# codename0og/codename-rvc-fork-3

Hardware: AMD Instinct MI355X
Metric: 48 kHz audio samples/sec end-to-end VC (higher is better)
Workload: dtype f32 (vocoder ResBlock convs and upsamplers, HuBERT, RMVPE's U-Net convs: fp32 operands as exact bf16x3 splits on the bf16 matrix cores -- six products of order <= 2^-16 per multiply-add, fp32 accumulate; everything else fp32 / fp64)

## Files before the change

codename-rvc-fork-3_amd/csrc/conv.h:

```cpp
#pragma once
#include <vector>

#include "common.h"

namespace rvc {

struct ConvParams {
    const float *x1 = nullptr; int c1 = 0; float slope1 = 1.f; int64_t x1_bstride = 0;
    const float *x2 = nullptr; int c2 = 0; float slope2 = 1.f; int64_t x2_bstride = 0;
    int64_t l_in = 0;
    int64_t l_in2 = 0;
    const float *w = nullptr;
    const uint16_t *w16 = nullptr;
    const float *bias = nullptr;
    int64_t bias_bstride = 0;
    const float *res = nullptr;
    const float *accin = nullptr;
    float *y = nullptr;
    int64_t y_bstride = 0;
    int m_total = 0;
    int c_out = 0;
    int64_t n_cols = 0;
    int64_t l_out = 0;
    int kw = 1, dil = 1, padl = 0;
    int up_stride = 0, up_pad = 0;
    int up_interleave = 0;
    float out_scale = 1.f;
    int batch = 1;
    const uint32_t *w_wino16 = nullptr;
    const void *w_f16x2 = nullptr;
    const void *w_direct1 = nullptr;
    const void *w_winobf = nullptr;
    const float *w_wino = nullptr;
    int debug = 0;
};

struct ConcurrencyScope {
    explicit ConcurrencyScope(int hint);
    ~ConcurrencyScope();
    int saved;
};

int launch_conv(const ConvParams &p, hipStream_t stream);

bool resblock_layer_supported(int c, int k);
int launch_resblock_layer(const float *x, const float *w1, const float *b1, const float *w2, const float *b2, const float *accin,
                          float *y, int batch, int c, int64_t L, int k, int dil, float slope, float out_scale, hipStream_t stream);

bool resblock_bf_enabled();
void resblock_bf_set_enabled(bool on);
bool resblock_bf_supported(int c, int k, int dil);
bool resblock_bf_preferred(int c, int k, int tap_splits = 3);
bool resblock_bf_fits(int c, int64_t L);
size_t resblock_bf_weight_bytes(int c, int k, int tap_splits = 3);
void resblock_bf_pack_host(const float *w1, const float *w2, int c, int k, std::vector<uint16_t> *out, int tap_splits = 3);
int launch_resblock_bf(const float *x, const void *u, const float *b1, const float *b2, const float *accin, float *y, int batch, int c,
                       int64_t L, int k, int dil, float slope, float out_scale, hipStream_t stream, int tap_splits = 3);

enum Cb1Format {
    CB1_BF16W = 0,
    CB1_F16X2 = 1,
};
bool convbf1_supported(int c, int k, int dil);
bool convbf1_preferred(Cb1Format fmt, int c, int k);
bool convbf1_fits(int c, int64_t L);
size_t convbf1_weight_bytes(Cb1Format fmt, int c, int k);
int convbf1_pack_host(Cb1Format fmt, const float *w, int c, int k, std::vector<uint16_t> *out);
int launch_convbf1(Cb1Format fmt, const float *x, const void *u, const float *bias, const float *res, const float *accin, float *y, int batch,
                   int c, int64_t L, int k, int dil, float slope, float out_scale, hipStream_t stream);

bool upsbf_supported(int c_in, int c_out, int rate, int ksize, int vk);
bool upsbf_fold_noise(int nc_k);
size_t upsbf_weight_bytes(int c_in, int c_out, int rate, int vk);
void upsbf_pack_host(const float *uw, const float *nw, const float *bias, int c_in, int c_out, int rate, int ksize, int vk, int nc_k,
                     int nc_stride, std::vector<uint16_t> *out);
int launch_upsbf(const float *x, const float *har, int64_t Lh, const void *u, const float *bias, float *y, int batch, int c_in, int c_out,
                 int64_t L_in, int64_t L_out, int rate, int ksize, int pad, int vk, int64_t S, int64_t P, float slope, hipStream_t stream);

bool conv2dbf_supported(int c_in, int c_out, int H, int W, int taps);
size_t conv2dbf_weight_bytes(int c_out, int c_in);
size_t conv2dbf_workspace_bytes(int batch, int c_in, int c_out, int H, int W);
void conv2dbf_pack_host(const float *w, int c_out, int c_in, std::vector<uint16_t> *out);
int launch_conv2dbf(const float *x, const void *u, const float *bias, const float *res, float *y, int batch, int c_in, int c_out, int H, int W,
                    int relu, float *ws, size_t ws_bytes, hipStream_t stream);
int launch_conv2d_finish(const float *partial, int split, int batch, int c_out, int H, int W, const float *bias, const float *res, int relu,
                         float *y, hipStream_t stream);

static inline uint16_t bf16_rne(float f) {
    uint32_t u;
    memcpy(&u, &f, 4);
    if ((u & 0x7fffffffu) > 0x7f800000u) return (uint16_t)((u >> 16) | 0x40);
    return (uint16_t)((u + 0x7fffu + ((u >> 16) & 1u)) >> 16);
}
static inline void bf16_split_host(float v, int n_terms, uint16_t *out) {
    for (int s = 0; s < n_terms; ++s) {
        out[s] = bf16_rne(v);
        const uint32_t bits = (uint32_t)out[s] << 16;
        float f;
        memcpy(&f, &bits, 4);
        v -= f;
    }
}

bool wino_enabled();
bool wino_supported(int k, int dil);
bool wino_fits(int c_in, int c_out, int64_t L);
int launch_wino_conv(const float *x, const void *u, bool u_bf16, const float *bias, const float *res, const float *accin, float *y,
                     int batch, int c_in, int c_out, int64_t L, int k, int dil, float slope, float out_scale, hipStream_t stream);
void wino_pack_host(const float *w_host, int c_out, int c_in, int k, std::vector<float> *out);
void wino_pack_host_bf16(const float *w_host, int c_out, int c_in, int k, std::vector<uint32_t> *out);

bool winobf_enabled();
bool winobf_supported(int c_in, int c_out, int k, int dil);
bool winobf_fits(int c_in, int c_out, int64_t L);
size_t winobf_weight_bytes(int c_out, int c_in, int k);
void winobf_pack_host(const float *w_host, int c_out, int c_in, int k, std::vector<uint16_t> *out);
int launch_winobf_conv(const float *x, const void *u, const float *bias, const float *res, const float *accin, float *y, int batch,
                       int c_in, int c_out, int64_t L, int k, int dil, float slope, float out_scale, hipStream_t stream);
bool winobf2_enabled();
bool winobf2_supported(int c_in, int c_out, int k, int dil);
int launch_winobf2_conv(const float *x, const void *u, const float *bias, const float *res, const float *accin, float *y, int batch,
                        int c_in, int c_out, int64_t L, int k, int dil, float slope, float out_scale, hipStream_t stream);

void conv_pack_host(const float *w_host, int c_out, int c_in, int k, std::vector<float> *out);

}
```

codename-rvc-fork-3_amd/csrc/conv.hip:

```cpp
#include <stdlib.h>

#include <atomic>

#include "conv.h"

namespace rvc {

constexpr int CONV_CH_ALIGN = 8;
constexpr int CONV_MAX_DIL = 5;

template <int KW, int MT, int NT, int WM, int WN, int CONV_CIC, bool UP, bool WB16 = false>
__global__ void __launch_bounds__(WM *WN * 64) __attribute__((amdgpu_waves_per_eu(MT == 1 ? 2 : 3, MT == 1 ? 2 : 3)))
conv_mfma_kernel(const ConvParams p) {
    constexpr int BM = 32 * MT * WM;
    constexpr int BN = 32 * NT * WN;
    constexpr int NTH = 64 * WM * WN;
    constexpr int XW = BN + (KW - 1) * CONV_MAX_DIL;
    constexpr int XTOT = CONV_CIC * XW;
    constexpr int XN = (XTOT + NTH - 1) / NTH;
    constexpr int W4TOT = KW * CONV_CIC * BM / 4;
    constexpr int WN4 = (W4TOT + NTH - 1) / NTH;

    constexpr int WTOT = KW * CONV_CIC * BM;
    __shared__ __attribute__((aligned(16))) float ws[2 * WTOT];
// ... 231 lines not shown
            }
#pragma unroll
            for (int m = 0; m < MT; ++m)
#pragma unroll
                for (int r = 0; r < 16; ++r)
#pragma unroll
                    for (int n = 0; n < NT; ++n)
                        if (ok[n]) *reinterpret_cast<float *>(reinterpret_cast<char *>(y) + boff(m, r, n)) = acc[m][n][r] * out_scale;
        }
    } else {
        const int c_out = p.c_out, up_stride = p.up_stride, up_pad = p.up_pad;
        const int64_t n_cols = p.n_cols, l_out = p.l_out;
        const float out_scale = p.out_scale;
        const int64_t cbase = col0 + wn * NT * 32 + l31;
        const float *bsrc = bias ? bias : p.w;
        if (p.up_interleave) {
            typedef float f32x2u __attribute__((ext_vector_type(2), aligned(4)));
            typedef float f32x4u __attribute__((ext_vector_type(4), aligned(4)));
            const bool quad = (up_stride & 3) == 0;
#pragma unroll
            for (int m = 0; m < MT; ++m)
#pragma unroll
                for (int r = 0; r < 16; r += 2) {
                    const int row = m0 + wm * MT * 32 + m * 32 + mfma32_row(r, lane);
                    const int co = row / up_stride, ph = row - co * up_stride;
                    float bv = bsrc[co];
                    bv = bias ? bv : 0.f;
                    float *q = y + (int64_t)co * l_out + ph - up_pad;
#pragma unroll
                    for (int n = 0; n < NT; ++n) {
                        const int64_t col = cbase + n * 32;
                        const int64_t t = col * up_stride + ph - up_pad;
                        const float v0 = (acc[m][n][r] + bv) * out_scale, v1 = (acc[m][n][r + 1] + bv) * out_scale;
                        if (col >= n_cols) continue;
                        if (quad) {
                            if ((r & 2) == 0) {
                                const float v2 = (acc[m][n][r + 2] + bv) * out_scale, v3 = (acc[m][n][r + 3] + bv) * out_scale;
                                if (t >= 0 && t + 3 < l_out) {
                                    *reinterpret_cast<f32x4u *>(q + col * up_stride) = f32x4u{v0, v1, v2, v3};
                                } else {
                                    const float vv[4] = {v0, v1, v2, v3};
#pragma unroll
                                    for (int e = 0; e < 4; ++e)
                                        if (t + e >= 0 && t + e < l_out) q[col * up_stride + e] = vv[e];
                                }
                            }
                        } else if (t >= 0 && t + 1 < l_out) {
                            *reinterpret_cast<f32x2u *>(q + col * up_stride) = f32x2u{v0, v1};
                        } else {
                            if (t >= 0 && t < l_out) q[col * up_stride] = v0;
                            if (t + 1 >= 0 && t + 1 < l_out) q[col * up_stride + 1] = v1;
                        }
                    }
                }
            return;
        }
#pragma unroll
        for (int m = 0; m < MT; ++m)
#pragma unroll
            for (int r = 0; r < 16; ++r) {
                const int row = m0 + wm * MT * 32 + m * 32 + mfma32_row(r, lane);
                const int phase = row / c_out;
                const int co = row - phase * c_out;
                float bv = bsrc[co];
                bv = bias ? bv : 0.f;
                float *q = y + (int64_t)co * l_out + phase - up_pad;
#pragma unroll
                for (int n = 0; n < NT; ++n) {
                    const int64_t col = cbase + n * 32;
                    const int64_t t = col * up_stride + phase - up_pad;
                    if (col < n_cols && t >= 0 && t < l_out) q[col * up_stride] = (acc[m][n][r] + bv) * out_scale;
                }
            }
    }
}

static std::atomic<int> g_concurrency{1};
static thread_local int t_concurrency = 0;
static int concurrency_hint() { return t_concurrency > 0 ? t_concurrency : g_concurrency.load(std::memory_order_relaxed); }
ConcurrencyScope::ConcurrencyScope(int hint) : saved(t_concurrency) { if (hint > 0) t_concurrency = hint; }
ConcurrencyScope::~ConcurrencyScope() { t_concurrency = saved; }

template <int KW, int MT, int NT, int WM, int WN, int CIC>
static int launch_cfg(const ConvParams &p, hipStream_t stream) {
    constexpr int BM = 32 * MT * WM;
    constexpr int BN = 32 * NT * WN;
    dim3 grid((unsigned)ceil_div(p.n_cols, BN), (unsigned)(p.m_total / BM), (unsigned)p.batch);
    if (p.up_stride > 0) {
        if constexpr (KW == 2) {
            hipLaunchKernelGGL((conv_mfma_kernel<KW, MT, NT, WM, WN, CIC, true>), grid, dim3(64 * WM * WN), 0, stream, p);
        } else {
            return fail("conv: scatter mode is built for 2-tap (polyphase) kernels only, got %d taps", KW);
        }
    } else if (p.w16) {
        if constexpr ((KW == 3 && CIC == 8) || ((KW == 7 || KW == 11) && CIC == 4)) {
            hipLaunchKernelGGL((conv_mfma_kernel<KW, MT, NT, WM, WN, CIC, false, true>), grid, dim3(64 * WM * WN), 0, stream, p);
        } else {
            return fail("conv: no bf16-weight kernel for %d taps at chunk depth %d", KW, CIC);
        }
    } else {
        hipLaunchKernelGGL((conv_mfma_kernel<KW, MT, NT, WM, WN, CIC, false>), grid, dim3(64 * WM * WN), 0, stream, p);
    }
    RVC_LAUNCH_CHECK();
    return 0;
}


template <int KW, int MT, int NT, int WM, int WN>
static int launch_cic(const ConvParams &p, hipStream_t stream, int cic) {
#ifdef RVC_ABLATE
    if (cic == 4) return launch_cfg<KW, MT, NT, WM, WN, 4>(p, stream);
    return launch_cfg<KW, MT, NT, WM, WN, 8>(p, stream);
#else
    (void)cic;
    return launch_cfg<KW, MT, NT, WM, WN, (KW >= 7 ? 4 : 8)>(p, stream);
#endif
}

template <int KW>
static int launch_kw(const ConvParams &p, hipStream_t stream) {
    static const int cic_env = knob("RVC_CONV_CIC", 0);
    int cic = KW >= 7 ? 4 : 8;
    if (cic_env && !p.w16) cic = cic_env;
    if ((p.c1 % cic) || (p.c2 % cic)) cic = 8;
    if (p.m_total % 128 == 0) {
        static const int narrow_env = knob("RVC_CONV_NARROW", 1);
        const int64_t tiles = ceil_div(p.n_cols, 128) * (p.m_total / 128) * p.batch;
        if (narrow_env && tiles < 1536 && concurrency_hint() <= 1) return launch_cic<KW, 2, 1, 2, 2>(p, stream, cic);
        return launch_cic<KW, 2, 2, 2, 2>(p, stream, cic);
    }
    if (p.m_total % 64 == 0) return launch_cic<KW, 2, 2, 1, 4>(p, stream, cic);
    if (p.m_total % 32 == 0) return launch_cic<KW, 1, 4, 1, 4>(p, stream, cic);
    return fail("conv: GEMM rows (%d) must be a multiple of 32", p.m_total);
}

bool wino_enabled() {
    static const int mode = knob("RVC_WINO", 1);
    return mode != 0;
}

bool winobf_enabled() {
    static const int mode = knob("RVC_WINOBF", 1);
    return mode != 0;
}

int launch_conv(const ConvParams &p_in, hipStream_t stream) {
    const bool plain = !p_in.x2 && p_in.up_stride == 0 && p_in.bias_bstride == 0 &&
        p_in.l_in == p_in.l_out && p_in.n_cols == p_in.l_out && p_in.x1_bstride == (int64_t)p_in.c1 * p_in.l_in &&
        p_in.y_bstride == (int64_t)p_in.m_total * p_in.l_out && p_in.slope1 >= 0.f && p_in.slope1 <= 1.f && p_in.padl == (p_in.kw - 1) / 2 * p_in.dil;
    if ((p_in.w_f16x2 || p_in.w_direct1) && plain && p_in.c1 == p_in.m_total && p_in.x1 != p_in.y && convbf1_supported(p_in.c1, p_in.kw, p_in.dil) &&
        convbf1_fits(p_in.c1, p_in.l_in))
        return launch_convbf1(p_in.w_f16x2 ? CB1_F16X2 : CB1_BF16W, p_in.x1, p_in.w_f16x2 ? p_in.w_f16x2 : p_in.w_direct1, p_in.bias, p_in.res, p_in.accin,
                              p_in.y, p_in.batch, p_in.c1, p_in.l_out, p_in.kw, p_in.dil, p_in.slope1, p_in.out_scale, stream);
    if (p_in.w_winobf && plain && wino_enabled() && winobf_enabled() && winobf_supported(p_in.c1, p_in.m_total, p_in.kw, p_in.dil) &&
        winobf_fits(p_in.c1, p_in.m_total, p_in.l_in))
        return launch_winobf_conv(p_in.x1, p_in.w_winobf, p_in.bias, p_in.res, p_in.accin, p_in.y, p_in.batch, p_in.c1, p_in.m_total, p_in.l_out,
                                  p_in.kw, p_in.dil, p_in.slope1, p_in.out_scale, stream);
    if ((p_in.w_wino || p_in.w_wino16) && !p_in.x2 && p_in.up_stride == 0 && p_in.c1 == p_in.m_total && p_in.bias_bstride == 0 &&
        p_in.l_in == p_in.l_out && p_in.n_cols == p_in.l_out && p_in.x1_bstride == (int64_t)p_in.c1 * p_in.l_in &&
        p_in.y_bstride == (int64_t)p_in.m_total * p_in.l_out && p_in.c1 % 32 == 0 && p_in.slope1 >= 0.f && p_in.slope1 <= 1.f && p_in.padl == (p_in.kw - 1) / 2 * p_in.dil &&
        wino_enabled() && wino_supported(p_in.kw, p_in.dil) && wino_fits(p_in.c1, p_in.m_total, p_in.l_in))
        return launch_wino_conv(p_in.x1, p_in.w_wino16 ? (const void *)p_in.w_wino16 : (const void *)p_in.w_wino, p_in.w_wino16 != nullptr, p_in.bias, p_in.res, p_in.accin, p_in.y, p_in.batch, p_in.c1, p_in.m_total, p_in.l_out,
                                p_in.kw, p_in.dil, p_in.slope1, p_in.out_scale, stream);
    static const int dbg = knob("RVC_CONV_DEBUG", 0);
    ConvParams p = p_in;
    p.debug = dbg;
    if ((p.c1 % CONV_CH_ALIGN) || (p.c2 % CONV_CH_ALIGN) || p.c1 + p.c2 <= 0)
        return fail("conv: input channels (%d + %d) must be multiples of %d", p.c1, p.c2, CONV_CH_ALIGN);
    if (p.dil < 1 || p.dil > CONV_MAX_DIL) return fail("conv: dilation %d out of range 1..%d", p.dil, CONV_MAX_DIL);
    if (p.n_cols <= 0 || p.batch <= 0) return 0;
    if (p.up_stride == 0 && (int64_t)p.m_total * p.l_out >= ((int64_t)1 << 30))
        return fail("conv: one output slab of %d x %lld floats exceeds the 4 GB the epilogue addresses", p.m_total,
                    (long long)p.l_out);
    switch (p.kw) {
        case 1: return launch_kw<1>(p, stream);
        case 2: return launch_kw<2>(p, stream);
        case 3: return launch_kw<3>(p, stream);
        case 5: return launch_kw<5>(p, stream);
        case 7: return launch_kw<7>(p, stream);
        case 11: return launch_kw<11>(p, stream);
        default: return fail("conv: unsupported kernel size %d (1, 2, 3, 5, 7, 11)", p.kw);
    }
}

void conv_pack_host(const float *w_host, int c_out, int c_in, int k, std::vector<float> *out) {
    out->resize((size_t)c_out * c_in * k);
    for (int co = 0; co < c_out; ++co)
        for (int ci = 0; ci < c_in; ++ci)
            for (int t = 0; t < k; ++t) (*out)[((size_t)t * c_in + ci) * c_out + co] = w_host[((size_t)co * c_in + ci) * k + t];
}

}

using namespace rvc;

extern "C" int rvc_set_concurrency_hint(int utterances_in_flight) {
    if (utterances_in_flight < 1) return fail("rvc_set_concurrency_hint: need at least 1, got %d", utterances_in_flight);
    g_concurrency.store(utterances_in_flight, std::memory_order_relaxed);
    return 0;
}

extern "C" int rvc_conv1d_pack_weight(const float *w_host, int c_out, int c_in, int k, float *w_packed_dev,
                                      void *stream) {
    if (!w_host || !w_packed_dev || c_out <= 0 || c_in <= 0 || k <= 0) return fail("rvc_conv1d_pack_weight: bad argument");
    std::vector<float> packed;
    conv_pack_host(w_host, c_out, c_in, k, &packed);
    return upload_packed("rvc_conv1d_pack_weight", packed.data(), packed.size() * sizeof(float), w_packed_dev, stream);
}

extern "C" int rvc_conv1d_forward(const float *x_dev, const float *w_packed_dev, const float *bias_dev,
                                  const float *res_dev, const float *acc_dev, float *y_dev, int batch, int c_in,
                                  int c_out, int64_t length, int k, int dilation, float slope_in, float out_scale,
                                  void *stream) {
    if (!x_dev || !w_packed_dev || !y_dev) return fail("rvc_conv1d_forward: null pointer");
    if (!(k & 1)) return fail("rvc_conv1d_forward: kernel size must be odd, got %d", k);
    ConvParams p;
    p.x1 = x_dev; p.c1 = c_in; p.slope1 = slope_in; p.x1_bstride = (int64_t)c_in * length;
    p.l_in = length;
    p.w = w_packed_dev; p.bias = bias_dev; p.res = res_dev; p.accin = acc_dev;
    p.y = y_dev; p.y_bstride = (int64_t)c_out * length;
    p.m_total = c_out; p.c_out = c_out; p.n_cols = length; p.l_out = length;
    p.kw = k; p.dil = dilation; p.padl = (k - 1) / 2 * dilation;
    p.out_scale = out_scale; p.batch = batch;
    return launch_conv(p, (hipStream_t)stream);
}
```

codename-rvc-fork-3_amd/csrc/convbf1.hip:

```cpp
#include <stdlib.h>

#include <algorithm>
#include <mutex>
#include <type_traits>
#include <vector>

#include "conv.h"
#include "f16x2.h"

namespace rvc {

constexpr int CB1_NTH = 512;
constexpr int CB1_CK = 64;
constexpr int CB1_N1 = 64;

struct Cb1Bf16Taps {
    static constexpr const char *NAME = "convbf1";
    using frag = bf16x8;
    static constexpr bool PAIRS = false;
    static constexpr int PLANES = 3;
    static constexpr int TAPF = 1;
    static constexpr int NACC = 1;
    static constexpr int OUT_OPS = 24, VM_MAX = 56;
    static constexpr int tap_plane(int) { return 0; }
    static constexpr int win_plane(int i) { return 2 - i; }
    static constexpr int acc_of(int) { return 0; }
};
struct Cb1F16Pairs {
    static constexpr const char *NAME = "convh2";
    using frag = f16x8;
    static constexpr bool PAIRS = true;
    static constexpr int PLANES = 2;
    static constexpr int TAPF = 2;
    static constexpr int NACC = 2;
    static constexpr int OUT_OPS = 28, VM_MAX = 60;
    static constexpr int tap_plane(int i) { return i == 2; }
    static constexpr int win_plane(int i) { return i == 0; }
    static constexpr int acc_of(int i) { return i != 1; }
};

struct Cb1Params {
    const float *x = nullptr;
    const void *u = nullptr;
    const float *bias = nullptr;
    const float *res = nullptr;
    const float *accin = nullptr;
    float *y = nullptr;
    int64_t L = 0;
    int dil = 1;
    float slope = 1.f, out_scale = 1.f;
    int tiles_per_row = 0, n_tiles = 0, per_xcd = 0;
};

template <int KW, int C, class F>
struct Cb1Geom {
    static constexpr int NCH = C / CB1_CK;
    static constexpr int RBW = C / 128;
    static constexpr int KS = CB1_CK / 16;
    static constexpr int NGC = KW * KS;
    static constexpr int NGT = NCH * NGC;
    static constexpr int H = (KW - 1) / 2;
    static constexpr int ROWB = 2 * F::PLANES * CB1_CK + 16;
    static constexpr int XROWS = CB1_N1 + (KW - 1) * 5;
    static constexpr int X_BYTES = (XROWS + 1) * ROWB;
    static constexpr int RC32 = (XROWS + 31) / 32;
    static constexpr int NIT = (CB1_CK / 8) * RC32 / 4;
    static constexpr int IO_BYTES = C * CB1_N1 * 4;
    static constexpr int LDS_BYTES = 2 * X_BYTES + IO_BYTES;
    static constexpr int ROWBLOCKS = C / 32;
    static constexpr int CONV_BYTES = NGT * ROWBLOCKS * F::TAPF * 1024;
    static constexpr int PA = F::TAPF == 1 ? 8 : 8 / RBW;
    static_assert(C == 128 || C == 256, "square layers of 128 or 256 channels");
    static_assert((CB1_CK / 8) * RC32 % 4 == 0, "the items must divide over the four stager waves");
    static_assert(4 * NIT + F::OUT_OPS <= F::VM_MAX, "memory operations in flight per stager wave");
    static_assert(LDS_BYTES <= 163840, "LDS budget");
    static_assert((ROWB / 16) % 2 == 1, "row stride must be an odd multiple of 16 bytes");
};

template <int KW, int C, class F>
__global__ void __launch_bounds__(CB1_NTH) __attribute__((amdgpu_waves_per_eu(2, 2)))
convbf1_kernel(const Cb1Params p) {
    using GM = Cb1Geom<KW, C, F>;
    using frag = typename F::frag;
    constexpr int NCH = GM::NCH, RBW = GM::RBW, KS = GM::KS, NGC = GM::NGC, NGT = GM::NGT, H = GM::H, ROWB = GM::ROWB, NIT = GM::NIT;
    constexpr int N1 = CB1_N1, CK = CB1_CK, PA = GM::PA, PLANES = F::PLANES, TAPF = F::TAPF, NACC = F::NACC;

    extern __shared__ __attribute__((aligned(16))) unsigned char cb_smem[];
    unsigned char *const xs = cb_smem;
    float *const io_lds = reinterpret_cast<float *>(cb_smem + 2 * GM::X_BYTES);

    const int tid = threadIdx.x, lane = tid & 63;
    const int wave = __builtin_amdgcn_readfirstlane(tid >> 6);
    const int half = lane >> 5, l31 = lane & 31;
    const int d = p.dil, XR = N1 + (KW - 1) * d;
    const int64_t L = p.L;
    const unsigned L4 = (unsigned)(L * 4);
    const int num_bytes = (int)((int64_t)C * L * 4);

    const int xcd = blockIdx.x & 7, slot = blockIdx.x >> 3, nslot = gridDim.x >> 3;
    const int tile_end = (xcd + 1) * p.per_xcd < p.n_tiles ? (xcd + 1) * p.per_xcd : p.n_tiles;
    const int tile0 = xcd * p.per_xcd + slot;
    if (tile0 >= tile_end) return;
    const int my_tiles = (tile_end - tile0 + nslot - 1) / nslot;
    const int n_q = my_tiles * NCH;

    if (wave >= 4) {
        __builtin_amdgcn_s_setprio(1);
        const int sw = wave - 4;
        float xr[NIT][4];
        constexpr int RC = GM::RC32;
        const int lq = lane >> 5;
        auto x_issue = [&](int q) __attribute__((always_inline)) {
            const int tl = tile0 + (q / NCH) * nslot, ch0 = (q % NCH) * CK;
            const int bb = tl / p.tiles_per_row;
            const int xt0 = (tl - bb * p.tiles_per_row) * N1 - H * d;
            const __amdgpu_buffer_rsrc_t rs = __builtin_amdgcn_make_buffer_rsrc((void *)(p.x + (int64_t)bb * C * L), 0, num_bytes, RSRC_RAW32);
            const unsigned Lu = (unsigned)L;
            int sw_o = sw;
            asm volatile("" : "+s"(sw_o));
#pragma unroll
            for (int i = 0; i < NIT; ++i) {
                const int wi = sw_o * NIT + i, qp = wi / RC, rc = wi - qp * RC;
                const int qd = 2 * qp + lq, r = rc * 32 + l31;
                const unsigned tg = (unsigned)(xt0 + r);
                const bool ok = r < XR && tg < Lu;
                const unsigned base = (unsigned)(ch0 + 4 * qd) * L4 + tg * 4u;
#pragma unroll
                for (int e = 0; e < 4; ++e)
                    xr[i][e] = __builtin_bit_cast(float, __builtin_amdgcn_raw_buffer_load_b32(rs, (int)(ok ? base + (unsigned)e * L4 : BUF_OOB), 0, 0));
            }
        };
        const float slope = p.slope;
        auto x_write = [&](int q) __attribute__((always_inline)) {
            unsigned char *const xb = xs + (q & 1) * GM::X_BYTES;
            int sw_o = sw;
            asm volatile("" : "+s"(sw_o));
#pragma unroll
            for (int i = 0; i < NIT; ++i) {
                const int wi = sw_o * NIT + i, qp = wi / RC, rc = wi - qp * RC;
                const int qd = 2 * qp + lq, r = rc * 32 + l31;
                unsigned w[2][PLANES];
#pragma unroll
                for (int e2 = 0; e2 < 2; ++e2) {
                    const float va = xr[i][2 * e2], vb = xr[i][2 * e2 + 1];
                    const float la = __builtin_fmaxf(va, mul_np(va, slope)), lb = __builtin_fmaxf(vb, mul_np(vb, slope));
                    if constexpr (F::PAIRS) split_f16x2_np(la, lb, w[e2][0], w[e2][1]);
                    else split3_np(la, lb, w[e2]);
                }
                unsigned char *o = xb + (r < XR ? r : GM::XROWS) * ROWB + qd * 8;
#pragma unroll
                for (int s = 0; s < PLANES; ++s) *reinterpret_cast<u32x2 *>(o + s * 2 * CK) = u32x2{w[0][s], w[1][s]};
                if (i & 1) __builtin_amdgcn_sched_barrier(0);
            }
        };
        constexpr int CHUNKS = N1 / 4, RPW = 64 / CHUNKS, PASSES = C / (4 * RPW);
        constexpr int HP = 4, NHF = PASSES / HP;
        const int chunk = lane % CHUNKS, rsub = lane / CHUNKS;
        const float out_scale = p.out_scale;
        const bool l4 = (L & 3) == 0;
        const bool has_res = p.res != nullptr, has_acc = p.accin != nullptr, has_bias = p.bias != nullptr;
        const __amdgpu_buffer_rsrc_t brs = __builtin_amdgcn_make_buffer_rsrc((void *)(has_bias ? p.bias : p.y), 0, C * 4, RSRC_RAW32);
        auto out_store = [&](int tl) __attribute__((always_inline)) {
            const int bb = tl / p.tiles_per_row;
            const int64_t t0 = (int64_t)(tl - bb * p.tiles_per_row) * N1;
            const bool ok = t0 + 4 * chunk < L;
            const __amdgpu_buffer_rsrc_t yrs = __builtin_amdgcn_make_buffer_rsrc((void *)(p.y + (int64_t)bb * C * L), 0, num_bytes, RSRC_RAW32);
            const __amdgpu_buffer_rsrc_t rrs = __builtin_amdgcn_make_buffer_rsrc((void *)((has_res ? p.res : p.y) + (int64_t)bb * C * L), 0, num_bytes, RSRC_RAW32);
            const __amdgpu_buffer_rsrc_t ars = __builtin_amdgcn_make_buffer_rsrc((void *)((has_acc ? p.accin : p.y) + (int64_t)bb * C * L), 0, num_bytes, RSRC_RAW32);
            const unsigned o0 = ok ? (unsigned)(sw * RPW + rsub) * L4 + (unsigned)(t0 + 4 * chunk) * 4u : BUF_OOB;
            auto load4 = [&](const __amdgpu_buffer_rsrc_t &rsrc, unsigned o) __attribute__((always_inline)) -> f32x4 {
                if (l4) return __builtin_bit_cast(f32x4, __builtin_amdgcn_raw_buffer_load_b128(rsrc, (int)o, 0, 0));
                float ae[4];
#pragma unroll
                for (int e = 0; e < 4; ++e) {
                    const unsigned oe = (ok && t0 + 4 * chunk + e < L) ? o + 4u * (unsigned)e : BUF_OOB;
                    ae[e] = __builtin_bit_cast(float, __builtin_amdgcn_raw_buffer_load_b32(rsrc, (int)oe, 0, 0));
                }
                return f32x4{ae[0], ae[1], ae[2], ae[3]};
            };
#pragma unroll
            for (int hf = 0; hf < NHF; ++hf) {
                f32x4 v[HP], rv[HP], av[HP];
                float bv[HP];
#pragma unroll
                for (int k = 0; k < HP; ++k) {
                    const unsigned o = o0 + (unsigned)((hf * HP + k) * 4 * RPW) * L4;
                    rv[k] = f32x4{0.f, 0.f, 0.f, 0.f};
                    av[k] = f32x4{0.f, 0.f, 0.f, 0.f};
                    if constexpr (F::PAIRS)
                        bv[k] = __builtin_bit_cast(float, __builtin_amdgcn_raw_buffer_load_b32(brs, (int)(has_bias ? (unsigned)((((hf * HP + k) * 4 + sw) * RPW + rsub) * 4) : BUF_OOB), 0, 0));
                    if (has_res) rv[k] = load4(rrs, o);
                    if (has_acc) av[k] = load4(ars, o);
                }
#pragma unroll
                for (int k = 0; k < HP; ++k) v[k] = *reinterpret_cast<const f32x4 *>(io_lds + (((hf * HP + k) * 4 + sw) * RPW + rsub) * N1 + 4 * chunk);
#pragma unroll
                for (int k = 0; k < HP; ++k) {
                    const unsigned o = o0 + (unsigned)((hf * HP + k) * 4 * RPW) * L4;
                    float re[4] = {v[k].x, v[k].y, v[k].z, v[k].w};
                    const float r4[4] = {rv[k].x, rv[k].y, rv[k].z, rv[k].w}, a4[4] = {av[k].x, av[k].y, av[k].z, av[k].w};
#pragma unroll
                    for (int e = 0; e < 4; ++e) {
                        if constexpr (F::PAIRS) re[e] = add_np(re[e], bv[k]);
                        if (has_res) re[e] = add_np(re[e], r4[e]);
                        if (has_acc) re[e] = add_np(re[e], a4[e]);
                        re[e] = mul_np(re[e], out_scale);
                    }
                    if (l4) {
                        __builtin_amdgcn_raw_buffer_store_b128(__builtin_bit_cast(u32x4, f32x4{re[0], re[1], re[2], re[3]}), yrs, (int)o, 0, 0);
                    } else {
#pragma unroll
                        for (int e = 0; e < 4; ++e) {
                            const unsigned oe = (ok && t0 + 4 * chunk + e < L) ? o + 4u * (unsigned)e : BUF_OOB;
                            __builtin_amdgcn_raw_buffer_store_b32(__builtin_bit_cast(unsigned, re[e]), yrs, (int)oe, 0, 0);
                        }
                    }
                }
            }
        };
        x_issue(0);
        x_write(0);
        if (1 < n_q) x_issue(1);
        for (int q = 0; q < n_q; ++q) {
            lds_barrier();
            if (q % NCH == 0 && q > 0) out_store(tile0 + (q / NCH - 1) * nslot);
            if (q + 1 < n_q) x_write(q + 1);
            asm volatile("s_waitcnt vmcnt(8)" ::: "memory");
            if (q + 2 < n_q) x_issue(q + 2);
        }
        lds_barrier();
        out_store(tile0 + (my_tiles - 1) * nslot);
        return;
    }

    float bias[RBW][16];
    if constexpr (!F::PAIRS) {
#pragma unroll
        for (int rb = 0; rb < RBW; ++rb)
#pragma unroll
            for (int r = 0; r < 16; ++r) {
                const int ch = 32 * (RBW * wave + rb) + (r & 3) + 8 * (r >> 2) + 4 * half;
                bias[rb][r] = p.bias ? p.bias[ch] : 0.f;
            }
    }
    const __amdgpu_buffer_rsrc_t urs = __builtin_amdgcn_make_buffer_rsrc((void *)p.u, 0, GM::CONV_BYTES, RSRC_RAW32);
    frag fa[PA][RBW][TAPF];
    frag fb[2][2][PLANES];
    f32x16 acc[RBW][2][NACC];
    auto load_a = [&](int slot_a, int g) __attribute__((always_inline)) {
        const int soff = (g * GM::ROWBLOCKS + RBW * wave) * TAPF * 1024;
#pragma unroll
        for (int f = 0; f < TAPF * RBW; ++f)
            fa[slot_a][f / TAPF][f % TAPF] = __builtin_bit_cast(frag, __builtin_amdgcn_raw_buffer_load_b128(urs, 16 * lane + f * 1024, soff, 0));
    };
    auto load_a1 = [&](int slot_a, int g, int f) __attribute__((always_inline)) {
        const int soff = (g * GM::ROWBLOCKS + RBW * wave) * TAPF * 1024;
        fa[slot_a][f / TAPF][f % TAPF] = __builtin_bit_cast(frag, __builtin_amdgcn_raw_buffer_load_b128(urs, 16 * lane + f * 1024, soff, 0));
    };
    auto load_b1 = [&](int buf, const unsigned char *src, int gc, int cb, int s) __attribute__((always_inline)) {
        const int tap = gc / KS, ks = gc - tap * KS;
        fb[buf][cb][s] = __builtin_bit_cast(frag, *reinterpret_cast<const u32x4 *>(src + tap * d * ROWB + ks * 32 + cb * 32 * ROWB + s * 2 * CK));
    };
#pragma unroll
    for (int g = 0; g < PA - 1; ++g) load_a(g, g);
    const int x_lane = l31 * ROWB + half * 16;
    float *const io_mine = io_lds + (32 * RBW * wave + 4 * half) * N1 + l31;
    constexpr int NM = 6 * RBW;

    static_assert((2 * NGC) % PA == 0 && NCH % 2 == 0, "two chunks of groups must be whole turns of the tap ring");
    int q = 0;
    for (int t = 0; t < my_tiles; ++t) {
#pragma unroll
        for (int rb = 0; rb < RBW; ++rb)
#pragma unroll
            for (int cb = 0; cb < 2; ++cb)
#pragma unroll
                for (int a = 0; a < NACC; ++a)
#pragma unroll
                    for (int r = 0; r < 16; ++r) acc[rb][cb][a][r] = 0.f;
#pragma unroll 1
        for (int cp = 0; cp < NCH / 2; ++cp) {
            const int g0 = cp * 2 * NGC;
#pragma unroll
            for (int c2 = 0; c2 < 2; ++c2, ++q) {
                lds_barrier();
                const unsigned char *const src = xs + (q & 1) * GM::X_BYTES + x_lane;
#pragma unroll
                for (int k = 0; k < 2 * PLANES; ++k) load_b1(0, src, 0, k & 1, PLANES - 1 - (k >> 1));
#pragma unroll
                for (int gc = 0; gc < NGC; ++gc) {
                    const int gl = c2 * NGC + gc;
#pragma unroll
                    for (int i = 0; i < 3; ++i)
#pragma unroll
                        for (int cb = 0; cb < 2; ++cb)
#pragma unroll
                            for (int rb = 0; rb < RBW; ++rb) {
                                const int k = (2 * i + cb) * RBW + rb;
                                const int wp = F::tap_plane(i), xp = F::win_plane(i), ap = F::acc_of(i);
                                if constexpr (F::PAIRS)
                                    acc[rb][cb][ap] = __builtin_amdgcn_mfma_f32_32x32x16_f16(fa[gl % PA][rb][wp], fb[gc & 1][cb][xp], acc[rb][cb][ap], 0, 0, 0);
                                else
                                    acc[rb][cb][ap] = __builtin_amdgcn_mfma_f32_32x32x16_bf16(fa[gl % PA][rb][wp], fb[gc & 1][cb][xp], acc[rb][cb][ap], 0, 0, 0);
                                __builtin_amdgcn_sched_barrier(0);
                                if (k < 2 * PLANES && gc + 1 < NGC) load_b1((gc + 1) & 1, src, gc + 1, k & 1, PLANES - 1 - (k >> 1));
                                if (k >= NM - TAPF * RBW) {
                                    int gn = g0 + gl + PA - 1;
                                    gn = gn >= NGT ? gn - NGT : gn;
                                    load_a1((gl + PA - 1) % PA, gn, k - (NM - TAPF * RBW));
                                }
                                __builtin_amdgcn_sched_barrier(0);
                            }
                }
            }
        }
#pragma unroll
        for (int rb = 0; rb < RBW; ++rb)
#pragma unroll
            for (int cb = 0; cb < 2; ++cb)
#pragma unroll
                for (int r = 0; r < 16; ++r)
                    if constexpr (F::PAIRS)
                        io_mine[(32 * rb + (r & 3) + 8 * (r >> 2)) * N1 + cb * 32] = __builtin_fmaf(acc[rb][cb][1][r], F16X2_LO_UNSCALE, acc[rb][cb][0][r]);
                    else
                        io_mine[(32 * rb + (r & 3) + 8 * (r >> 2)) * N1 + cb * 32] = acc[rb][cb][0][r] + bias[rb][r];
    }
    lds_barrier();
}


bool convbf1_supported(int c, int k, int dil) { return (c == 128 || c == 256) && (k == 3 || k == 7 || k == 11) && dil >= 1 && dil <= 5; }

bool convbf1_preferred(Cb1Format fmt, int c, int k) {
    if (fmt == CB1_F16X2) {
#ifdef RVC_ABLATE
        static const int on = knob("RVC_CH2", 1);
        if (!on) return false;
#endif
        return convbf1_supported(c, k, 1);
    }
#ifdef RVC_ABLATE
    static const int on = knob("RVC_CB1", 1);
    if (!on) return false;
    static const int all = knob("RVC_CB1_ALL", 0);
    if (all) return true;
#endif
    return (c == 128 && k == 11) || c == 256;
}

bool convbf1_fits(int c, int64_t L) { return fits_2gib((int64_t)c * L, 4); }

size_t convbf1_weight_bytes(Cb1Format fmt, int c, int k) { return (size_t)(c / 16) * k * (c / 32) * 1024 * (fmt == CB1_F16X2 ? 2 : 1); }

int convbf1_pack_host(Cb1Format fmt, const float *w, int c, int k, std::vector<uint16_t> *out) {
    const int NCH = c / CB1_CK, KS = CB1_CK / 16, RB = c / 32, planes = fmt == CB1_F16X2 ? 2 : 1;
    if (fmt == CB1_F16X2)
        for (size_t i = 0, n = (size_t)c * c * k; i < n; ++i)
            if (!(w[i] >= -F16_MAX && w[i] <= F16_MAX)) return 1;
    out->assign(convbf1_weight_bytes(fmt, c, k) / 2, 0);
    for (int ch = 0; ch < NCH; ++ch)
        for (int tap = 0; tap < k; ++tap)
            for (int ks = 0; ks < KS; ++ks)
                for (int rb = 0; rb < RB; ++rb)
                    for (int lane = 0; lane < 64; ++lane)
                        for (int e = 0; e < 8; ++e) {
                            const int co = 32 * rb + (lane & 31), ci = CB1_CK * ch + 16 * ks + 8 * (lane >> 5) + e;
                            const size_t group = ((size_t)ch * k + tap) * KS + ks, at = (group * RB + rb) * planes * 512 + lane * 8 + e;
                            const float v = w[((size_t)co * c + ci) * k + tap];
                            if (fmt == CB1_F16X2) f16x2_split_host(v, &(*out)[at], &(*out)[at + 512]);
                            else (*out)[at] = bf16_rne(v);
                        }
    return 0;
}

template <int KW, int C, class F>
static int cb1_launch(Cb1Params p, int batch, hipStream_t stream) {
    if (reserve_whole_cu((const void *)convbf1_kernel<KW, C, F>, F::NAME)) return 1;
    p.tiles_per_row = (int)ceil_div(p.L, CB1_N1);
    p.n_tiles = p.tiles_per_row * batch;
    const PersistentGrid g = persistent_grid(p.n_tiles);
    p.per_xcd = g.per_xcd;
    hipLaunchKernelGGL((convbf1_kernel<KW, C, F>), dim3(g.blocks), dim3(CB1_NTH), LDS_WHOLE_CU, stream, p);
    RVC_LAUNCH_CHECK();
    return 0;
}

template <class F>
static int cb1_dispatch(const Cb1Params &p, int batch, int c, int k, hipStream_t stream) {
#define RVC_CB1_CASE(KW, CC) if (k == KW && c == CC) return cb1_launch<KW, CC, F>(p, batch, stream)
    RVC_CB1_CASE(3, 128); RVC_CB1_CASE(7, 128); RVC_CB1_CASE(11, 128);
    RVC_CB1_CASE(3, 256); RVC_CB1_CASE(7, 256); RVC_CB1_CASE(11, 256);
#undef RVC_CB1_CASE
    return fail("%s: unsupported shape c=%d k=%d", F::NAME, c, k);
}

int launch_convbf1(Cb1Format fmt, const float *x, const void *u, const float *bias, const float *res, const float *accin, float *y, int batch,
                   int c, int64_t L, int k, int dil, float slope, float out_scale, hipStream_t stream) {
    const char *const name = fmt == CB1_F16X2 ? Cb1F16Pairs::NAME : Cb1Bf16Taps::NAME;
    if (!convbf1_supported(c, k, dil)) return fail("%s: unsupported shape (%d channels, %d taps, dilation %d)", name, c, k, dil);
    if (x == y) return fail("%s: in-place operation is not supported", name);
    if (!(slope >= 0.f && slope <= 1.f)) return fail("%s: leaky slope %g outside [0, 1]", name, (double)slope);
    if (!convbf1_fits(c, L)) return fail("%s: a %d x %lld slab exceeds the 2 GiB buffer addressing", name, c, (long long)L);
    if (L <= 0 || batch <= 0) return 0;
    if ((int64_t)ceil_div(L, CB1_N1) * batch >= ((int64_t)1 << 28)) return fail("%s: too many tiles", name);
    Cb1Params p;
    p.x = x; p.u = u; p.bias = bias; p.res = res; p.accin = accin; p.y = y; p.L = L; p.dil = dil; p.slope = slope; p.out_scale = out_scale;
    return fmt == CB1_F16X2 ? cb1_dispatch<Cb1F16Pairs>(p, batch, c, k, stream) : cb1_dispatch<Cb1Bf16Taps>(p, batch, c, k, stream);
}

}

using namespace rvc;


static int cb1_abi_weight_bytes(Cb1Format fmt, const char *fn, int c, int k, size_t *bytes) {
    if (!bytes) return fail("%s: null pointer", fn);
    if (!convbf1_supported(c, k, 1)) return fail("%s: c must be 128 or 256, k 3, 7 or 11", fn);
    *bytes = convbf1_weight_bytes(fmt, c, k);
    return 0;
}

static int cb1_abi_pack_weight(Cb1Format fmt, const char *fn, const char *shape_fn, const float *w_host, int c, int k, void *u_dev, void *stream) {
    if (!w_host || !u_dev) return fail("%s: null pointer", fn);
    size_t bytes = 0;
    if (cb1_abi_weight_bytes(fmt, shape_fn, c, k, &bytes)) return 1;
    std::vector<uint16_t> u;
    if (convbf1_pack_host(fmt, w_host, c, k, &u)) return fail("%s: a tap is non-finite or beyond +-65504, the range of an fp16 pair", fn);
    return upload_packed(fn, u.data(), bytes, u_dev, stream);
}

static int cb1_abi_forward(Cb1Format fmt, const char *fn, const float *x_dev, const void *u_dev, const float *bias_dev, const float *res_dev,
                           const float *acc_dev, float *y_dev, int batch, int c, int64_t length, int k, int dilation, float slope_in,
                           float out_scale, void *stream) {
    if (!x_dev || !u_dev || !y_dev) return fail("%s: null pointer", fn);
    return launch_convbf1(fmt, x_dev, u_dev, bias_dev, res_dev, acc_dev, y_dev, batch, c, length, k, dilation, slope_in, out_scale,
                          (hipStream_t)stream);
}

extern "C" int rvc_conv1d_bf16w_weight_bytes(int c, int k, size_t *bytes) {
    return cb1_abi_weight_bytes(CB1_BF16W, "rvc_conv1d_bf16w_weight_bytes", c, k, bytes);
}
extern "C" int rvc_conv1d_bf16w_pack_weight(const float *w_host, int c, int k, void *u_dev, void *stream) {
    return cb1_abi_pack_weight(CB1_BF16W, "rvc_conv1d_bf16w_pack_weight", "rvc_conv1d_bf16w_weight_bytes", w_host, c, k, u_dev, stream);
}
extern "C" int rvc_conv1d_bf16w_forward(const float *x_dev, const void *u_dev, const float *bias_dev, const float *res_dev,
                                        const float *acc_dev, float *y_dev, int batch, int c, int64_t length, int k, int dilation,
                                        float slope_in, float out_scale, void *stream) {
    return cb1_abi_forward(CB1_BF16W, "rvc_conv1d_bf16w_forward", x_dev, u_dev, bias_dev, res_dev, acc_dev, y_dev, batch, c, length, k,
                           dilation, slope_in, out_scale, stream);
}

extern "C" int rvc_conv1d_f16x2_weight_bytes(int c, int k, size_t *bytes) {
    return cb1_abi_weight_bytes(CB1_F16X2, "rvc_conv1d_f16x2_weight_bytes", c, k, bytes);
}
extern "C" int rvc_conv1d_f16x2_pack_weight(const float *w_host, int c, int k, void *u_dev, void *stream) {
    return cb1_abi_pack_weight(CB1_F16X2, "rvc_conv1d_f16x2_pack_weight", "rvc_conv1d_f16x2_pack_weight", w_host, c, k, u_dev, stream);
}
extern "C" int rvc_conv1d_f16x2_forward(const float *x_dev, const void *u_dev, const float *bias_dev, const float *res_dev,
                                        const float *acc_dev, float *y_dev, int batch, int c, int64_t length, int k, int dilation,
                                        float slope_in, float out_scale, void *stream) {
    return cb1_abi_forward(CB1_F16X2, "rvc_conv1d_f16x2_forward", x_dev, u_dev, bias_dev, res_dev, acc_dev, y_dev, batch, c, length, k,
                           dilation, slope_in, out_scale, stream);
}
```

codename-rvc-fork-3_amd/csrc/decoder.h:

```cpp
#pragma once
#include <atomic>
#include <map>
#include <mutex>
#include <string>
#include <vector>

#include "conv.h"

namespace rvc {

constexpr int MRF_MAX_DIM = 9;

struct HostTensor {
    std::vector<float> data;
    std::vector<int64_t> shape;
    int64_t numel() const { int64_t n = 1; for (auto s : shape) n *= s; return n; }
};

template <typename T>
struct DevBufT {
    T *p = nullptr;
    ~DevBufT() { if (p) (void)hipFree(p); }
    int upload(const std::vector<T> &h) {
        if (p) { (void)hipFree(p); p = nullptr; }
        hipError_t e = hipMalloc((void **)&p, h.size() * sizeof(T));
        if (e == hipSuccess) e = hipMemcpy(p, h.data(), h.size() * sizeof(T), hipMemcpyHostToDevice);
        return e == hipSuccess ? 0 : fail("device upload of %zu %zu-byte values failed: %s", h.size(), sizeof(T), hipGetErrorString(e));
    }
};
using DevBuf = DevBufT<float>;
using DevBuf16 = DevBufT<uint16_t>;

struct ConvW {
    DevBuf w, b;
    DevBuf16 w16;
    DevBuf wu;
    DevBuf16 wu16;
    DevBuf16 wx;
    DevBuf16 wd;
    DevBuf16 wh;
    int c_in = 0, c_out = 0, k = 0;
};

struct Stage {
    int c_in = 0, c_out = 0, rate = 0, ksize = 0, pad = 0, opad = 0;
    int taps = 0;
    bool interleave = false;
    int nc_stride = 0, nc_k = 0, nc_pad = 0;
    int vk = 0, vk_rows = 0;
    int64_t S = 0, P = 0;
    DevBuf w, b;
    DevBuf16 wub;
    int ub_vk = 0;
    int nc_rows = 0;
    DevBuf nc_w;
    std::vector<ConvW> c1, c2;
    std::vector<DevBuf16> pair;
    int pair_splits = 3;
};

constexpr int MAX_BRANCH_LANES = 7;
struct BranchLanes {
    hipStream_t side[MAX_BRANCH_LANES] = {};
    hipEvent_t fork = nullptr;
    hipEvent_t last[MAX_BRANCH_LANES + 1] = {};
    int n_side = 0;
    int create(int n);
    ~BranchLanes();
};

struct RefineStage {
    int ch_in = 0, ch_out = 0, rate = 0, down_c = 0, down_k = 0, down_stride = 0, down_pad = 0;
    DevBuf down_w, down_b;
    ConvW input_conv;
    DevBuf adain1[4], adain2[4];
    std::vector<ConvW> c1, c2;
    std::vector<DevBuf16> pair;
};

}

struct rvc_decoder {
    rvc_decoder_config cfg;
    std::map<std::string, rvc::HostTensor> host;
    bool finalized = false;
    int arithmetic = 0;
    int upp = 1;
    int dim = 1;
    float lin_w[rvc::MRF_MAX_DIM] = {0};
    float lin_b = 0.f;
    rvc::ConvW pre;
    rvc::DevBuf cond_w, cond_b;
    std::vector<rvc::Stage> stages;
    rvc::DevBuf post_w;
    float post_b = 0.f;
    int post_cin = 0;
    float merge_w = 1.f;
    rvc::DevBuf pre_w, pre_b;
    rvc::ConvW mel;
    std::vector<rvc::RefineStage> rstages;
    std::atomic<int> concurrency{0};
    std::atomic<int> branch_parallel{0};
    std::mutex lanes_mu;
    std::map<hipStream_t, rvc::BranchLanes *> lanes;
    ~rvc_decoder() { for (auto &kv : lanes) delete kv.second; }
    int tap_stage = -2;
    float *tap_dev = nullptr;
};


namespace rvc {
const HostTensor *find(const rvc_decoder *d, const std::string &name);
int need(const rvc_decoder *d, const std::string &name, const HostTensor **out, std::vector<int64_t> shape);
int build_conv(const rvc_decoder *d, const std::string &prefix, int c_out, int c_in, int k, bool bias, ConvW *out, bool as_bf16 = false);

int launch_unfold_src(const float *har, int batch, int64_t L, int64_t S, int64_t P, int k_valid, int k_rows, int64_t nq, float *V,
                      hipStream_t stream);
int launch_cond_bias(const float *pre_b, const float *cond_w, const float *cond_b, const float *g, int batch, int gin, int c0,
                     float *out, hipStream_t stream);
int launch_conv_post(const float *x, const float *w, float bias, int batch, int c_in, int64_t L, float slope, float *out,
                     hipStream_t stream, int64_t o_lo = 0, int64_t n_out = -1);

int refine_finalize(rvc_decoder *d);
size_t refine_workspace_bytes(const rvc_decoder *d, int batch, int64_t T);
int refine_forward(rvc_decoder *d, const float *z_dev, const float *f0_dev, const float *g_dev, const rvc_decoder_noise *noise,
                   int batch, int64_t T, float *out_dev, void *workspace_dev, size_t workspace_bytes, hipStream_t stream);
}
```

codename-rvc-fork-3_amd/csrc/decoder.hip:

```cpp
#include <stdlib.h>

#include "decoder.h"

namespace rvc {


constexpr int CARRY_CHUNK = 4096;
__global__ void __launch_bounds__(256)
nsf_carry_kernel(const float *__restrict__ f0, int64_t T, float sr, float upp, float *__restrict__ carry) {
    __shared__ double pre[CARRY_CHUNK];
    __shared__ double part[257];
    __shared__ double cum_s;
    constexpr int SEG = CARRY_CHUNK / 256;
    const int64_t b = blockIdx.x;
    const float *f = f0 + b * T;
    float *c = carry + b * T;
    if (threadIdx.x == 0) {
        c[0] = 0.f;
        cum_s = 0.0;
    }
    for (int64_t base = 0; base + 1 < T; base += CARRY_CHUNK) {
        const int n = (int)((T - 1 - base) < CARRY_CHUNK ? (T - 1 - base) : CARRY_CHUNK);
        for (int i = threadIdx.x; i < n; i += 256) {
            const float last = __fmul_rn(__fdiv_rn(f[base + i], sr), upp);
// ... 252 lines not shown
    const int64_t b = blockIdx.y;
    const int64_t t0 = o_lo + ((int64_t)blockIdx.x * blockDim.x + threadIdx.x) * POST_OUT;
    const int64_t blk0 = o_lo + (int64_t)blockIdx.x * blockDim.x * POST_OUT;
    const int64_t o_hi = o_lo + n_out;
    const float *xb = x + b * c_in * L;
    const bool fast = (L & 3) == 0 && (c_in & 3) == 0 && ((o_lo | n_out) & 3) == 0 && blk0 >= 4 &&
                      blk0 + (int64_t)blockDim.x * POST_OUT + 4 <= L && blk0 + (int64_t)blockDim.x * POST_OUT <= o_hi;
    if (fast) {
        float acc[POST_OUT];
#pragma unroll
        for (int o = 0; o < POST_OUT; ++o) acc[o] = bias;
        for (int c0 = 0; c0 < c_in; c0 += 4) {
            f32x4 q[4][3];
#pragma unroll
            for (int u = 0; u < 4; ++u) {
                const f32x4 *xr = reinterpret_cast<const f32x4 *>(xb + (int64_t)(c0 + u) * L + t0 - 4);
#pragma unroll
                for (int j = 0; j < 3; ++j) q[u][j] = xr[j];
            }
#pragma unroll
            for (int u = 0; u < 4; ++u) {
                float v[12];
#pragma unroll
                for (int j = 0; j < 3; ++j)
#pragma unroll
                    for (int e = 0; e < 4; ++e) v[4 * j + e] = q[u][j][e];
#pragma unroll
                for (int i = 1; i < 11; ++i) v[i] = lrelu(v[i], slope);
#pragma unroll
                for (int k = 0; k < 7; ++k) {
                    const float wk = w[(c0 + u) * 7 + k];
#pragma unroll
                    for (int o = 0; o < POST_OUT; ++o) acc[o] = fmaf(wk, v[o + k + 1], acc[o]);
                }
            }
        }
        *reinterpret_cast<f32x4 *>(out + b * n_out + (t0 - o_lo)) = f32x4{tanhf(acc[0]), tanhf(acc[1]), tanhf(acc[2]), tanhf(acc[3])};
        return;
    }
    if (t0 >= o_hi) return;
    float acc[POST_OUT];
#pragma unroll
    for (int o = 0; o < POST_OUT; ++o) acc[o] = bias;
    for (int ci = 0; ci < c_in; ++ci) {
        const float *xr = xb + (int64_t)ci * L;
        float v[POST_OUT + 6];
#pragma unroll
        for (int i = 0; i < POST_OUT + 6; ++i) {
            const int64_t tt = t0 + i - 3;
            const int64_t tc = tt < 0 ? 0 : (tt >= L ? L - 1 : tt);
            const float raw = xr[tc];
            v[i] = (tt >= 0 && tt < L) ? lrelu(raw, slope) : 0.f;
        }
#pragma unroll
        for (int k = 0; k < 7; ++k) {
            const float wk = w[ci * 7 + k];
#pragma unroll
            for (int o = 0; o < POST_OUT; ++o) acc[o] = fmaf(wk, v[o + k], acc[o]);
        }
    }
#pragma unroll
    for (int o = 0; o < POST_OUT; ++o)
        if (t0 + o < o_hi) out[b * n_out + (t0 - o_lo) + o] = tanhf(acc[o]);
}

int launch_unfold_src(const float *har, int batch, int64_t L, int64_t S, int64_t P, int k_valid, int k_rows, int64_t nq, float *V,
                      hipStream_t stream) {
    hipLaunchKernelGGL(unfold_src_kernel, dim3((unsigned)ceil_div(nq, 256), k_rows, batch), dim3(256), 0, stream, har, L, S, P,
                       k_valid, k_rows, nq, V);
    RVC_LAUNCH_CHECK();
    return 0;
}

int launch_cond_bias(const float *pre_b, const float *cond_w, const float *cond_b, const float *g, int batch, int gin, int c0,
                     float *out, hipStream_t stream) {
    hipLaunchKernelGGL(cond_bias_kernel, dim3(c0, batch), dim3(64), 0, stream, pre_b, cond_w, cond_b, g, gin, c0, out);
    RVC_LAUNCH_CHECK();
    return 0;
}

int launch_conv_post(const float *x, const float *w, float bias, int batch, int c_in, int64_t L, float slope, float *out,
                     hipStream_t stream, int64_t o_lo, int64_t n_out) {
    if (n_out < 0) n_out = L - o_lo;
    hipLaunchKernelGGL(conv_post_kernel, dim3((unsigned)ceil_div(n_out, 256 * POST_OUT), batch), dim3(256), 0, stream, x, w, bias, c_in, L,
                       o_lo, n_out, slope, out);
    RVC_LAUNCH_CHECK();
    return 0;
}


}

using namespace rvc;

namespace rvc {
const HostTensor *find(const rvc_decoder *d, const std::string &name) {
    auto it = d->host.find(name);
    return it == d->host.end() ? nullptr : &it->second;
}

int need(const rvc_decoder *d, const std::string &name, const HostTensor **out, std::vector<int64_t> shape) {
    const HostTensor *t = find(d, name);
    if (!t) return fail("decoder: tensor '%s' was never set", name.c_str());
    if (t->shape != shape) {
        std::string got, want;
        for (auto s : t->shape) got += std::to_string(s) + ",";
        for (auto s : shape) want += std::to_string(s) + ",";
        return fail("decoder: tensor '%s' has shape [%s], expected [%s]", name.c_str(), got.c_str(), want.c_str());
    }
    *out = t;
    return 0;
}

int build_conv(const rvc_decoder *d, const std::string &prefix, int c_out, int c_in, int k, bool bias, ConvW *out, bool as_bf16) {
    const HostTensor *w, *b;
    if (need(d, prefix + ".weight", &w, {c_out, c_in, k})) return 1;
    std::vector<float> packed;
    conv_pack_host(w->data.data(), c_out, c_in, k, &packed);
    if (as_bf16) {
        std::vector<uint16_t> half(packed.size());
        for (size_t i = 0; i < packed.size(); ++i) half[i] = bf16_rne(packed[i]);
        if (out->w16.upload(half)) return 1;
    } else if (out->w.upload(packed)) {
        return 1;
    }
    if (c_in == c_out && c_out % 32 == 0 && wino_supported(k, 1)) {
        if (as_bf16) {
            std::vector<uint32_t> words;
            wino_pack_host_bf16(w->data.data(), c_out, c_in, k, &words);
            std::vector<uint16_t> halves(words.size() * 2);
            memcpy(halves.data(), words.data(), words.size() * 4);
            if (out->wu16.upload(halves)) return 1;
            if (convbf1_supported(c_out, k, 1) && convbf1_preferred(CB1_BF16W, c_out, k)) {
                std::vector<uint16_t> frags;
                convbf1_pack_host(CB1_BF16W, w->data.data(), c_out, k, &frags);
                if (out->wd.upload(frags)) return 1;
            }
            if (winobf_enabled() && winobf_supported(c_in, c_out, k, 1)) {
                std::vector<float> vals((size_t)c_out * c_in * k);
                for (size_t i = 0; i < vals.size(); ++i) {
                    const uint32_t bits = (uint32_t)bf16_rne(w->data[i]) << 16;
                    memcpy(&vals[i], &bits, 4);
                }
                std::vector<uint16_t> frags;
                winobf_pack_host(vals.data(), c_out, c_in, k, &frags);
                if (out->wx.upload(frags)) return 1;
            }
        } else {
            wino_pack_host(w->data.data(), c_out, c_in, k, &packed);
            if (out->wu.upload(packed)) return 1;
            if (d->arithmetic == 1 && convbf1_supported(c_out, k, 1) && convbf1_preferred(CB1_F16X2, c_out, k)) {
                std::vector<uint16_t> frags;
                if (!convbf1_pack_host(CB1_F16X2, w->data.data(), c_out, k, &frags) && out->wh.upload(frags)) return 1;
            }
            if (winobf_enabled() && winobf_supported(c_in, c_out, k, 1)) {
                std::vector<uint16_t> frags;
                winobf_pack_host(w->data.data(), c_out, c_in, k, &frags);
                if (out->wx.upload(frags)) return 1;
            }
        }
    }
    if (c_in != c_out && !as_bf16 && k >= 7 && winobf_enabled() && winobf_supported(c_in, c_out, k, 1)) {
        std::vector<uint16_t> frags;
        winobf_pack_host(w->data.data(), c_out, c_in, k, &frags);
        if (out->wx.upload(frags)) return 1;
    }
    if (bias) {
        if (need(d, prefix + ".bias", &b, {c_out})) return 1;
        if (out->b.upload(b->data)) return 1;
    }
    out->c_in = c_in; out->c_out = c_out; out->k = k;
    return 0;
}
}

extern "C" int rvc_decoder_create(const rvc_decoder_config *cfg, rvc_decoder **out) {
    if (!cfg || !out) return fail("rvc_decoder_create: null pointer");
    if (cfg->kind != RVC_DEC_NSF && cfg->kind != RVC_DEC_MRF && cfg->kind != RVC_DEC_REFINE)
        return fail("rvc_decoder_create: unknown decoder kind %d", cfg->kind);
    if (cfg->n_ups < 1 || cfg->n_ups > 8) return fail("rvc_decoder_create: n_ups out of range");
    if (cfg->n_res_kernels < 1 || cfg->n_res_kernels > 4 || cfg->n_res_dilations < 1 || cfg->n_res_dilations > 4)
        return fail("rvc_decoder_create: resblock configuration out of range");
    if (cfg->weight_storage != 0 && cfg->weight_storage != 1) return fail("rvc_decoder_create: weight_storage must be 0 (fp32) or 1 (bf16)");
    if (cfg->weight_storage == 1 && cfg->kind == RVC_DEC_REFINE)
        return fail("rvc_decoder_create: bf16 weight storage is built for the NSF / MRF decoders (BASELINE cfg 4), not RefineGAN");
    if (cfg->in_channels % 8 || cfg->upsample_initial_channel % (32 << cfg->n_ups))
        return fail("rvc_decoder_create: channel counts must keep every stage a multiple of 32");
    rvc_decoder *d = new rvc_decoder();
    d->cfg = *cfg;
    d->upp = 1;
    for (int i = 0; i < cfg->n_ups; ++i) d->upp *= cfg->upsample_rates[i];
    if (d->upp > 1024) { delete d; return fail("rvc_decoder_create: prod(upsample_rates) > 1024"); }
    d->dim = cfg->kind == RVC_DEC_MRF ? 9 : 1;
    *out = d;
    return 0;
}

extern "C" int rvc_decoder_set_arithmetic(rvc_decoder *dec, int mode) {
    if (!dec) return fail("rvc_decoder_set_arithmetic: null decoder");
    if (mode != 0 && mode != 1) return fail("rvc_decoder_set_arithmetic: mode must be 0 (exact) or 1 (fp16 pairs), got %d", mode);
    if (dec->finalized) return fail("rvc_decoder_set_arithmetic: decoder already finalized (the tap slabs are packed at finalize)");
    if (mode == 1 && dec->cfg.weight_storage == 1)
        return fail("rvc_decoder_set_arithmetic: fp16 pairs are for fp32 taps; a weight_storage = 1 handle's bf16 taps already cost three products");
    dec->arithmetic = mode;
    return 0;
}

extern "C" int rvc_decoder_set_tensor(rvc_decoder *dec, const char *name, const float *data_host, const int64_t *shape,
                                      int ndim) {
    if (!dec || !name || !data_host || !shape || ndim < 1 || ndim > 4) return fail("rvc_decoder_set_tensor: bad argument");
    if (dec->finalized) return fail("rvc_decoder_set_tensor: decoder already finalized");
    HostTensor t;
    t.shape.assign(shape, shape + ndim);
    const int64_t n = t.numel();
    if (n <= 0) return fail("rvc_decoder_set_tensor: empty tensor '%s'", name);
    t.data.assign(data_host, data_host + n);
    dec->host[name] = std::move(t);
    return 0;
}

extern "C" int rvc_decoder_finalize(rvc_decoder *d) {
    if (!d) return fail("rvc_decoder_finalize: null decoder");
    if (d->finalized) return 0;
    if (d->cfg.kind == RVC_DEC_REFINE) {
        if (refine_finalize(d)) return 1;
        d->host.clear();
        d->finalized = true;
        return 0;
    }
    const rvc_decoder_config &c = d->cfg;
    const bool mrf = c.kind == RVC_DEC_MRF;
    const HostTensor *t;
    if (need(d, "m_source.l_linear.weight", &t, {1, d->dim})) return 1;
    for (int h = 0; h < d->dim; ++h) d->lin_w[h] = t->data[h];
    if (need(d, "m_source.l_linear.bias", &t, {1})) return 1;
    d->lin_b = t->data[0];
    const int c0 = c.upsample_initial_channel;
    if (build_conv(d, "conv_pre", c0, c.in_channels, 7, true, &d->pre)) return 1;
    if (need(d, "cond.weight", &t, {c0, c.gin_channels, 1})) return 1;
    if (d->cond_w.upload(t->data)) return 1;
    if (need(d, "cond.bias", &t, {c0})) return 1;
    if (d->cond_b.upload(t->data)) return 1;
    d->stages.clear();
    d->stages.resize(c.n_ups);
    for (int i = 0; i < c.n_ups; ++i) {
        Stage &s = d->stages[i];
        s.c_in = c0 >> i;
        s.c_out = c0 >> (i + 1);
        s.rate = c.upsample_rates[i];
        s.ksize = c.upsample_kernel_sizes[i];
        s.pad = (s.rate % 2 == 0) ? (s.ksize - s.rate) / 2 : s.rate / 2 + s.rate % 2;
        s.opad = s.rate % 2;
        s.taps = (s.ksize + s.rate - 1) / s.rate;
        if (s.taps > 2) return fail("decoder: upsample kernel %d with rate %d needs %d polyphase taps (max 2)", s.ksize, s.rate, s.taps);
        if (s.taps < 2) s.taps = 2;
        int stride_f0 = 1;
        for (int j = i + 1; j < c.n_ups; ++j) stride_f0 *= c.upsample_rates[j];
        s.nc_stride = stride_f0;
        s.nc_k = stride_f0 == 1 ? 1 : stride_f0 * 2 - stride_f0 % 2;
        s.nc_pad = stride_f0 == 1 ? 0 : (s.nc_k - stride_f0) / 2;
        s.vk = (s.rate - 1) * s.nc_stride + s.nc_k;
        s.vk_rows = (s.vk + 7) / 8 * 8;
        s.S = (int64_t)s.rate * s.nc_stride;
        s.P = (int64_t)s.pad * s.nc_stride + s.nc_pad;
        static const int nc_sep_env = knob("RVC_NC_SEPARATE", 1);
        const bool nc_separate = nc_sep_env && s.vk_rows * 2 >= s.c_in;
        if (nc_separate) {
            s.nc_rows = (s.nc_k + 7) / 8 * 8;
            s.vk = 0;
            s.vk_rows = 0;
        }

        const std::string up = (mrf ? "upsamples." : "ups.") + std::to_string(i);
        const std::string nc = "noise_convs." + std::to_string(i);
        const HostTensor *uw, *ub, *nw, *nb;
        if (need(d, up + ".weight", &uw, {s.c_in, s.c_out, s.ksize})) return 1;
        if (need(d, up + ".bias", &ub, {s.c_out})) return 1;
        if (need(d, nc + ".weight", &nw, {s.c_out, 1, s.nc_k})) return 1;
        if (need(d, nc + ".bias", &nb, {s.c_out})) return 1;
        const int ctot = s.c_in + s.vk_rows;
        const int m_total = s.rate * s.c_out;
        s.interleave = s.rate % 2 == 0;
        auto mrow = [&](int ph, int co) { return s.interleave ? co * s.rate + ph : ph * s.c_out + co; };
        std::vector<float> packed((size_t)s.taps * ctot * m_total, 0.f);
        for (int tp = 0; tp < s.taps; ++tp) {
            const int j = s.taps - 1 - tp;
            for (int ci = 0; ci < s.c_in; ++ci)
                for (int ph = 0; ph < s.rate; ++ph) {
                    const int kk = ph + j * s.rate;
                    if (kk >= s.ksize) continue;
                    for (int co = 0; co < s.c_out; ++co)
                        packed[((size_t)tp * ctot + ci) * m_total + mrow(ph, co)] =
                            uw->data[((size_t)ci * s.c_out + co) * s.ksize + kk];
                }
        }
        const int tp0 = s.taps - 1;
        for (int kq = 0; kq < s.vk; ++kq)
            for (int ph = 0; ph < s.rate; ++ph) {
                const int k = kq - ph * s.nc_stride;
                if (k < 0 || k >= s.nc_k) continue;
                for (int co = 0; co < s.c_out; ++co)
                    packed[((size_t)tp0 * ctot + s.c_in + kq) * m_total + mrow(ph, co)] = nw->data[(size_t)co * s.nc_k + k];
            }
        if (s.w.upload(packed)) return 1;
        std::vector<float> bias(s.c_out);
        for (int co = 0; co < s.c_out; ++co) bias[co] = ub->data[co] + nb->data[co];
// ... 216 lines not shown
    const int64_t L = Tw * d->upp;
    const float sr = (float)c.sample_rate;

    if (!mrf) {
        hipLaunchKernelGGL(nsf_carry_kernel, dim3(batch), dim3(256), 0, stream, f0_dev, T, sr, (float)d->upp, carry);
        RVC_LAUNCH_CHECK();
        hipLaunchKernelGGL(nsf_source_kernel, dim3((unsigned)ceil_div(L, 256), batch), dim3(256), 0, stream, f0_dev, carry,
                           noise->src_randn_dev, T, ext_lo, Tw, d->upp, sr, d->lin_w[0], d->lin_b, har);
        RVC_LAUNCH_CHECK();
    } else {
        MrfSrcParams sp;
        sp.f0 = f0_dev; sp.rand_ini = noise->src_rand_dev; sp.randn = noise->src_randn_dev; sp.har = har;
        sp.p1 = (double *)(ws + lay.p1); sp.p2 = (double *)(ws + lay.p2); sp.wraps = (int *)(ws + lay.wraps);
        sp.tot_unused = nullptr;
        sp.T = T; sp.upp = d->upp; sp.dim = d->dim; sp.sr = sr;
        sp.i0 = ext_lo; sp.Tw = Tw;
        for (int h = 0; h < MRF_MAX_DIM; ++h) sp.lin_w[h] = d->lin_w[h];
        sp.lin_b = d->lin_b;
        hipLaunchKernelGGL(mrf_prefix_kernel<1>, dim3(batch), dim3(256), 0, stream, sp);
        RVC_LAUNCH_CHECK();
        hipLaunchKernelGGL(mrf_wraps_kernel, dim3((unsigned)T, d->dim, batch), dim3(64), 0, stream, sp);
        RVC_LAUNCH_CHECK();
        hipLaunchKernelGGL(mrf_prefix_kernel<3>, dim3(batch), dim3(256), 0, stream, sp);
        RVC_LAUNCH_CHECK();
        hipLaunchKernelGGL(mrf_source_kernel, dim3((unsigned)Tw, batch), dim3(256), 0, stream, sp);
        RVC_LAUNCH_CHECK();
    }
    if (d->tap_stage == -1 && d->tap_dev)
        RVC_HIP(hipMemcpyAsync(d->tap_dev, har, (size_t)batch * L * 4, hipMemcpyDeviceToDevice, stream));

    const int c0 = c.upsample_initial_channel;
    hipLaunchKernelGGL(cond_bias_kernel, dim3(c0, batch), dim3(64), 0, stream, d->pre.b.p, d->cond_w.p, d->cond_b.p, g_dev,
                       c.gin_channels, c0, biasp);
    RVC_LAUNCH_CHECK();
    float *cur = buf[0];
    if (Tw != T) {
        RVC_HIP(hipMemcpy2DAsync(buf[1], (size_t)Tw * 4, z_dev + ext_lo, (size_t)T * 4, (size_t)Tw * 4, (size_t)batch * c.in_channels,
                                 hipMemcpyDeviceToDevice, stream));
        z_dev = buf[1];
    }
    {
        ConvParams p;
        p.x1 = z_dev; p.c1 = c.in_channels; p.slope1 = 1.f; p.x1_bstride = (int64_t)c.in_channels * Tw; p.l_in = Tw;
        p.w = d->pre.w.p; p.bias = biasp; p.bias_bstride = c0;
        p.y = cur; p.y_bstride = (int64_t)c0 * Tw; p.m_total = c0; p.c_out = c0; p.n_cols = Tw; p.l_out = Tw;
        p.kw = 7; p.dil = 1; p.padl = 3; p.batch = batch;
        if (launch_conv(p, stream)) return 1;
    }

    int64_t len = Tw;
    const int nd = c.n_res_dilations, nk = c.n_res_kernels;
    for (int i = 0; i < c.n_ups; ++i) {
        Stage &s = d->stages[i];
        const int64_t nq = len + 1;
        const int64_t len_out = (len - 1) * s.rate - 2 * s.pad + s.ksize + s.opad;
        float *X = buf[1];
        if (s.wub.p && fits_2gib((int64_t)s.c_in * len, 4) && fits_2gib((int64_t)s.c_out * len_out, 4) && fits_2gib(L, 4)) {
            if (launch_upsbf(cur, har, L, s.wub.p, s.b.p, X, batch, s.c_in, s.c_out, len, len_out, s.rate, s.ksize, s.pad, s.ub_vk, s.S, s.P, 0.1f, stream))
                return 1;
        } else {
        if (s.vk_rows) {
            hipLaunchKernelGGL(unfold_src_kernel, dim3((unsigned)ceil_div(nq, 256), s.vk_rows, batch), dim3(256), 0, stream, har, L,
                               s.S, s.P, s.vk, s.vk_rows, nq, V);
            RVC_LAUNCH_CHECK();
        }
        {
            ConvParams p;
            p.x1 = cur; p.c1 = s.c_in; p.slope1 = 0.1f; p.x1_bstride = (int64_t)s.c_in * len;
            if (s.vk_rows) { p.x2 = V; p.c2 = s.vk_rows; p.slope2 = 1.f; p.x2_bstride = (int64_t)s.vk_rows * nq; }
            p.l_in = len;
            p.w = s.w.p; p.bias = s.b.p;
            p.y = X; p.y_bstride = (int64_t)s.c_out * len_out;
            p.m_total = s.rate * s.c_out; p.c_out = s.c_out; p.n_cols = nq; p.l_out = len_out;
            p.kw = s.taps; p.dil = 1; p.padl = s.taps - 1;
            p.up_stride = s.rate; p.up_pad = s.pad; p.up_interleave = s.interleave ? 1 : 0; p.batch = batch;
            p.l_in2 = nq;
            if (launch_conv(p, stream)) return 1;
        }
        }
        if (s.nc_rows) {
            hipLaunchKernelGGL(unfold_src_kernel, dim3((unsigned)ceil_div(len_out, 256), s.nc_rows, batch), dim3(256), 0, stream, har,
                               L, (int64_t)s.nc_stride, (int64_t)s.nc_pad, s.nc_k, s.nc_rows, len_out, V);
            RVC_LAUNCH_CHECK();
            ConvParams p;
            p.x1 = V; p.c1 = s.nc_rows; p.slope1 = 1.f; p.x1_bstride = (int64_t)s.nc_rows * len_out; p.l_in = len_out;
            p.w = s.nc_w.p; p.accin = X; p.y = X; p.y_bstride = (int64_t)s.c_out * len_out;
            p.m_total = s.c_out; p.c_out = s.c_out; p.n_cols = len_out; p.l_out = len_out;
            p.kw = 1; p.dil = 1; p.padl = 0; p.batch = batch;
            if (launch_conv(p, stream)) return 1;
        }
        len = len_out;
        const int64_t bs = (int64_t)s.c_out * len;
        const bool short_stage = (int64_t)batch * bs <= BRANCH_PARALLEL_MAX_ELEMS;
        const bool par = lanes && short_stage;
        if (par) {
            RVC_HIP(hipEventRecord(lanes->fork, stream));
            for (int q = 0; q < n_side; ++q) RVC_HIP(hipStreamWaitEvent(lanes->side[q], lanes->fork, 0));
        }
        const hipStream_t main_stream = stream;
        for (int r = 0; r < nk; ++r) {
            const int m = r;
            const bool first_branch = r == 0, final_branch = r + 1 == nk;
            const int k = c.res_kernel_sizes[m];
            const float *xin = X;
            const int off = nk - 1 - n_side;
            const int lane = par && r > off ? r - off : 0, lane_prev = par && r - 1 > off ? r - 1 - off : 0;
            const hipStream_t stream = lane > 0 ? lanes->side[lane - 1] : main_stream;
            float *const Y = buf[2 + 2 * lane], *const T1 = buf[3 + 2 * lane];
            auto before_last = [&]() -> int {
                if (par && r > 0 && lane_prev != lane) RVC_HIP(hipStreamWaitEvent(stream, lanes->last[r - 1], 0));
                return 0;
            };
            auto after_last = [&]() -> int {
                if (par) RVC_HIP(hipEventRecord(lanes->last[r], stream));
                return 0;
            };
            bool f16_branch = true;
            for (int j = 0; j < nd; ++j) f16_branch = f16_branch && s.c1[m * nd + j].wh.p && s.c2[m * nd + j].wh.p;
            if (s.pair[m * nd].p && !f16_branch && resblock_bf_fits(s.c_out, len)) {
                for (int j = 0; j < nd; ++j) {
                    const bool last = j + 1 == nd;
                    float *yout = last ? cur : (j % 2 == 0 ? Y : T1);
                    const float *acc_in = (last && !first_branch) ? cur : nullptr;
                    const float scale = (last && final_branch) ? 1.f / (float)nk : 1.f;
                    if (last && before_last()) return 1;
                    if (launch_resblock_bf(xin, s.pair[m * nd + j].p, s.c1[m * nd + j].b.p, s.c2[m * nd + j].b.p, acc_in, yout, batch,
                                           s.c_out, len, k, c.res_dilations[j], 0.1f, scale, stream, s.pair_splits))
                        return 1;
                    xin = yout;
                }
                if (after_last()) return 1;
                continue;
            }
            if (resblock_layer_supported(s.c_out, k) && !s.c1[m * nd].w16.p) {
                for (int j = 0; j < nd; ++j) {
                    const bool last = j + 1 == nd;
                    float *yout = last ? cur : (j % 2 == 0 ? Y : T1);
                    const float *acc_in = (last && !first_branch) ? cur : nullptr;
                    const float scale = (last && final_branch) ? 1.f / (float)nk : 1.f;
                    if (last && before_last()) return 1;
                    if (launch_resblock_layer(xin, s.c1[m * nd + j].w.p, s.c1[m * nd + j].b.p, s.c2[m * nd + j].w.p,
                                              s.c2[m * nd + j].b.p, acc_in, yout, batch, s.c_out, len, k, c.res_dilations[j], 0.1f,
                                              scale, stream))
                        return 1;
                    xin = yout;
                }
                if (after_last()) return 1;
                continue;
            }
            for (int j = 0; j < nd; ++j) {
                const int dil = c.res_dilations[j];
                ConvParams p;
                p.x1 = xin; p.c1 = s.c_out; p.slope1 = 0.1f; p.x1_bstride = bs; p.l_in = len;
                p.w = s.c1[m * nd + j].w.p; p.w16 = s.c1[m * nd + j].w16.p; p.bias = s.c1[m * nd + j].b.p; p.w_wino = s.c1[m * nd + j].wu.p; p.w_winobf = s.c1[m * nd + j].wx.p; p.w_direct1 = s.c1[m * nd + j].wd.p; p.w_f16x2 = s.c1[m * nd + j].wh.p;
                p.w_wino16 = reinterpret_cast<const uint32_t *>(s.c1[m * nd + j].wu16.p);
                p.y = T1; p.y_bstride = bs; p.m_total = s.c_out; p.c_out = s.c_out; p.n_cols = len; p.l_out = len;
                p.kw = k; p.dil = dil; p.padl = (k - 1) / 2 * dil; p.batch = batch;
                if (launch_conv(p, stream)) return 1;
                ConvParams q;
                q.x1 = T1; q.c1 = s.c_out; q.slope1 = 0.1f; q.x1_bstride = bs; q.l_in = len;
                q.w = s.c2[m * nd + j].w.p; q.w16 = s.c2[m * nd + j].w16.p; q.bias = s.c2[m * nd + j].b.p; q.w_wino = s.c2[m * nd + j].wu.p; q.w_winobf = s.c2[m * nd + j].wx.p; q.w_direct1 = s.c2[m * nd + j].wd.p; q.w_f16x2 = s.c2[m * nd + j].wh.p;
                q.w_wino16 = reinterpret_cast<const uint32_t *>(s.c2[m * nd + j].wu16.p);
                q.res = xin;
                q.y_bstride = bs; q.m_total = s.c_out; q.c_out = s.c_out; q.n_cols = len; q.l_out = len;
                q.kw = k; q.dil = 1; q.padl = (k - 1) / 2;  q.batch = batch;
                if (j + 1 < nd) {
                    q.y = Y;
                } else {
                    q.y = cur;
                    q.accin = first_branch ? nullptr : cur;
                    q.out_scale = final_branch ? 1.f / (float)nk : 1.f;
                    if (before_last()) return 1;
                }
                if (launch_conv(q, stream)) return 1;
                xin = Y;
            }
            if (after_last()) return 1;
        }
        if (par) RVC_HIP(hipStreamWaitEvent(main_stream, lanes->last[nk - 1], 0));
        if (d->tap_stage == i && d->tap_dev)
            RVC_HIP(hipMemcpyAsync(d->tap_dev, cur, (size_t)batch * bs * 4, hipMemcpyDeviceToDevice, stream));
    }
    if (len != L) return fail("decoder: internal length mismatch (%lld vs %lld)", (long long)len, (long long)L);
    return launch_conv_post(cur, d->post_w.p, d->post_b, batch, d->post_cin, L, 0.01f, out_dev, stream, o_lo, n_out);
}
}

extern "C" int rvc_decoder_forward(rvc_decoder *d, const float *z_dev, const float *f0_dev, const float *g_dev,
                                   const rvc_decoder_noise *noise, int batch, int64_t T, float *out_dev,
                                   void *workspace_dev, size_t workspace_bytes, void *stream_) {
    if (!d || !z_dev || !f0_dev || !g_dev || !noise || !out_dev || !workspace_dev) return fail("rvc_decoder_forward: null pointer");
    ConcurrencyScope scope(d->concurrency.load(std::memory_order_relaxed));
    if (!d->finalized) return fail("rvc_decoder_forward: decoder not finalized");
    if (batch <= 0 || T <= 0) return fail("rvc_decoder_forward: empty batch");
    if (!noise->src_randn_dev) return fail("rvc_decoder_forward: src_randn_dev is required");
    if (d->cfg.kind == RVC_DEC_REFINE)
        return refine_forward(d, z_dev, f0_dev, g_dev, noise, batch, T, out_dev, workspace_dev, workspace_bytes, (hipStream_t)stream_);
    return decoder_run(d, z_dev, f0_dev, g_dev, noise, batch, T, 0, T, 0, T * d->upp, out_dev, workspace_dev, workspace_bytes,
                       (hipStream_t)stream_);
}

extern "C" int rvc_decoder_window_margin(const rvc_decoder_config *cfg, int *frames) {
    if (!cfg || !frames) return fail("rvc_decoder_window_margin: null pointer");
    if (cfg->kind != RVC_DEC_NSF && cfg->kind != RVC_DEC_MRF && cfg->kind != RVC_DEC_REFINE)
        return fail("rvc_decoder_window_margin: unknown decoder kind %d", cfg->kind);
    if (cfg->n_ups < 1 || cfg->n_ups > 8) return fail("rvc_decoder_window_margin: n_ups out of range");
    if (cfg->n_res_kernels < 1 || cfg->n_res_kernels > 4 || cfg->n_res_dilations < 1 || cfg->n_res_dilations > 4)
        return fail("rvc_decoder_window_margin: resblock configuration out of range");
    for (int i = 0; i < cfg->n_ups; ++i)
        if (cfg->upsample_rates[i] < 1 || cfg->upsample_kernel_sizes[i] < cfg->upsample_rates[i])
            return fail("rvc_decoder_window_margin: upsample stage %d: rate %d, kernel %d", i, cfg->upsample_rates[i], cfg->upsample_kernel_sizes[i]);
    *frames = cfg->kind == RVC_DEC_REFINE ? -1 : window_margin(*cfg);
    return 0;
}

extern "C" int rvc_decoder_forward_window(rvc_decoder *d, const float *z_dev, const float *f0_dev, const float *g_dev,
                                          const rvc_decoder_noise *noise, int batch, int64_t T, int64_t keep_lo, int64_t keep_hi,
                                          float *out_dev, void *workspace_dev, size_t workspace_bytes, void *stream_) {
    if (!d || !z_dev || !f0_dev || !g_dev || !noise || !out_dev || !workspace_dev) return fail("rvc_decoder_forward_window: null pointer");
    ConcurrencyScope scope(d->concurrency.load(std::memory_order_relaxed));
    if (!d->finalized) return fail("rvc_decoder_forward_window: decoder not finalized");
    if (batch <= 0 || T <= 0) return fail("rvc_decoder_forward_window: empty batch");
    if (keep_lo < 0 || keep_lo >= keep_hi || keep_hi > T)
        return fail("rvc_decoder_forward_window: frames [%lld, %lld) are not a window of [0, %lld)", (long long)keep_lo, (long long)keep_hi, (long long)T);
    if (!noise->src_randn_dev) return fail("rvc_decoder_forward_window: src_randn_dev is required");
    if (d->cfg.kind == RVC_DEC_REFINE)
        return fail("rvc_decoder_forward_window: RefineGAN's receptive field is not covered; use rvc_decoder_forward");
    if (d->tap_dev) return fail("rvc_decoder_forward_window: a debug tap is set (rvc_decoder_set_tap); use rvc_decoder_forward");
    const int64_t m = window_margin(d->cfg);
    const int64_t ext_lo = std::max<int64_t>(0, keep_lo - m), ext_hi = std::min<int64_t>(T, keep_hi + m);
    return decoder_run(d, z_dev, f0_dev, g_dev, noise, batch, T, ext_lo, ext_hi - ext_lo, (keep_lo - ext_lo) * d->upp,
                       (keep_hi - keep_lo) * d->upp, out_dev, workspace_dev, workspace_bytes, (hipStream_t)stream_);
}
```

codename-rvc-fork-3_amd/rvc_amd/_native.py:

```python
from __future__ import annotations

import ctypes
import threading
import os
from ctypes import POINTER, c_char_p, c_double, c_float, c_int, c_int64, c_size_t, c_void_p

import torch

_HERE = os.path.dirname(os.path.abspath(__file__))
LIB_PATH = os.path.join(_HERE, "_lib", "librvc_amd.so")
if os.environ.get("RVC_AMD_LIB"):
    LIB_PATH = os.path.abspath(os.environ["RVC_AMD_LIB"])
    print(f"[rvc_amd] RVC_AMD_LIB: loading {LIB_PATH} instead of the product library", flush=True)


class NativeError(RuntimeError):
    pass


if not os.path.isfile(LIB_PATH):
    raise ImportError(
        f"{LIB_PATH} is missing: build it with `python -c 'import __graft_entry__ as g; g.build()'` "
        "(hipcc --offload-arch=gfx950).  rvc_amd has no fallback path without its HIP library.")

_lib = ctypes.CDLL(LIB_PATH)


class DecoderConfig(ctypes.Structure):
    _fields_ = [
        ("kind", c_int), ("sample_rate", c_int), ("in_channels", c_int), ("upsample_initial_channel", c_int),
        ("gin_channels", c_int), ("n_ups", c_int), ("upsample_rates", c_int * 8), ("upsample_kernel_sizes", c_int * 8),
        ("n_res_kernels", c_int), ("res_kernel_sizes", c_int * 4), ("res_dilations", c_int * 4),
        ("n_res_dilations", c_int), ("weight_storage", c_int),
    ]


class DecoderNoise(ctypes.Structure):
    _fields_ = [("src_rand_dev", c_void_p), ("src_randn_dev", c_void_p), ("adain_randn_dev", c_void_p)]


SYMBOLS = {
    "rvc_abi_version": (c_int, []),
    "rvc_last_error": (c_char_p, []),
    "rvc_knn_index_aux_bytes": (c_int, [c_int64, c_int, POINTER(c_size_t)]),
    "rvc_knn_index_build": (c_int, [c_void_p, c_int64, c_int, c_void_p, c_size_t, c_void_p]),
    "rvc_knn_set_mode": (c_int, [c_int]),
    "rvc_knn_rank_candidates": (c_int, [c_void_p, c_void_p, c_int64, c_int, c_void_p, c_int64, c_void_p, c_int, c_int, c_void_p,
                                        c_void_p, c_void_p]),
    "rvc_knn_workspace_bytes": (c_int, [c_int64, c_int64, c_int, c_int, POINTER(c_size_t)]),
    "rvc_knn_search": (c_int, [c_void_p, c_void_p, c_int64, c_int, c_void_p, c_int64, c_int, c_void_p, c_void_p,
                               c_void_p, c_size_t, c_void_p]),
    "rvc_knn_blend": (c_int, [c_void_p, c_int, c_void_p, c_void_p, c_void_p, c_int64, c_int, c_float, c_void_p,
                              c_void_p]),
    "rvc_logmel_workspace_bytes": (c_int, [c_int, c_int64, POINTER(c_size_t)]),
    "rvc_logmel_rmvpe": (c_int, [c_void_p, c_int, c_int64, c_void_p, c_int64, c_void_p, c_size_t, c_void_p]),
    "rvc_mel_create": (c_int, [c_int, c_int, c_int, c_int, c_float, c_float, c_void_p, c_int, POINTER(c_void_p)]),
    "rvc_mel_destroy": (c_int, [c_void_p]),
    "rvc_mel_frames": (c_int, [c_void_p, c_int64, POINTER(c_int64)]),
    "rvc_mel_workspace_bytes": (c_int, [c_void_p, c_int, c_int64, POINTER(c_size_t)]),
    "rvc_mel_forward": (c_int, [c_void_p, c_void_p, c_int, c_int64, c_void_p, c_void_p, c_void_p, c_size_t, c_void_p]),
    "rvc_resample_poly_f64": (c_int, [c_void_p, c_int64, c_int, c_int, c_void_p, c_int64, c_void_p, c_int64, c_void_p]),
    "rvc_filtfilt_workspace_bytes": (c_int, [c_int64, POINTER(c_size_t)]),
    "rvc_filtfilt_order5": (c_int, [c_void_p, c_int64, c_void_p, c_void_p, c_void_p, c_size_t, c_void_p]),
    "rvc_bigru_workspace_bytes": (c_int, [c_int, POINTER(c_size_t)]),
    "rvc_bigru_forward": (c_int, [c_void_p, c_void_p, c_void_p, c_void_p, c_int, c_int64, c_int, c_void_p, c_size_t,
                                  c_void_p]),
    "rvc_bigru_status": (c_int, [c_void_p, c_int, POINTER(c_int), c_void_p]),
    "rvc_bigru_set_spin_limit": (c_int, [ctypes.c_uint]),
    "rvc_attention_workspace_bytes": (c_int, [c_int, c_int64, c_int, c_int, POINTER(c_size_t)]),
    "rvc_attention_qkv_f32": (c_int, [c_void_p, c_void_p, c_void_p, c_void_p, c_int, c_int64, c_int, c_int, c_float,
                                      c_void_p, c_size_t, c_void_p]),
    "rvc_bias_relu_add_f32": (c_int, [c_void_p, c_void_p, c_void_p, c_void_p, c_int, c_int, c_int64, c_int, c_void_p]),
    "rvc_gate_tanh_sigmoid_f32": (c_int, [c_void_p, c_void_p, c_int, c_int, c_int64, c_void_p]),
    "rvc_rownorm_gelu_f32": (c_int, [c_void_p, c_void_p, c_void_p, c_void_p, c_int, c_int, c_int64, ctypes.c_float, c_void_p]),
    "rvc_set_concurrency_hint": (c_int, [c_int]),
    "rvc_decoder_create": (c_int, [POINTER(DecoderConfig), POINTER(c_void_p)]),
    "rvc_decoder_set_tensor": (c_int, [c_void_p, c_char_p, c_void_p, POINTER(c_int64), c_int]),
    "rvc_decoder_finalize": (c_int, [c_void_p]),
    "rvc_decoder_destroy": (c_int, [c_void_p]),
    "rvc_decoder_upp": (c_int, [c_void_p]),
    "rvc_decoder_workspace_bytes": (c_int, [c_void_p, c_int, c_int64, POINTER(c_size_t)]),
    "rvc_decoder_forward": (c_int, [c_void_p, c_void_p, c_void_p, c_void_p, POINTER(DecoderNoise), c_int, c_int64,
                                    c_void_p, c_void_p, c_size_t, c_void_p]),
    "rvc_decoder_window_margin": (c_int, [POINTER(DecoderConfig), POINTER(c_int)]),
    "rvc_decoder_forward_window": (c_int, [c_void_p, c_void_p, c_void_p, c_void_p, POINTER(DecoderNoise), c_int, c_int64, c_int64,
                                           c_int64, c_void_p, c_void_p, c_size_t, c_void_p]),
    "rvc_decoder_set_tap": (c_int, [c_void_p, c_int, c_void_p]),
    "rvc_decoder_set_concurrency_hint": (c_int, [c_void_p, c_int]),
    "rvc_decoder_set_branch_parallel": (c_int, [c_void_p, c_int]),
    "rvc_posconv_bf16x3_weight_bytes": (c_int, [c_int, c_int, c_int, POINTER(c_size_t)]),
    "rvc_posconv_bf16x3_pack_weight": (c_int, [c_void_p, c_int, c_int, c_int, c_void_p, c_void_p]),
    "rvc_posconv_gelu_bf16x3": (c_int, [c_void_p, c_void_p, c_void_p, c_void_p, c_int64, c_int, c_int, c_int, c_int, c_void_p]),
    "rvc_hubert_conv0_workspace_bytes": (c_int, [c_int, POINTER(c_size_t)]),
    "rvc_hubert_conv0_frames_bf16x3": (c_int, [c_void_p, c_int64, c_void_p, c_int, c_int, c_int, c_void_p, c_void_p, c_float, c_void_p,
                                               c_size_t, c_void_p, c_int64, c_void_p]),
    "rvc_conv1d_frames_bf16x3": (c_int, [c_void_p, c_int64, c_int64, c_int, c_int, c_int, c_void_p, c_void_p, c_void_p, c_void_p, c_int64,
                                         c_int, c_int, c_void_p]),
    "rvc_conv1d_pack_weight": (c_int, [c_void_p, c_int, c_int, c_int, c_void_p, c_void_p]),
    "rvc_conv1d_forward": (c_int, [c_void_p, c_void_p, c_void_p, c_void_p, c_void_p, c_void_p, c_int, c_int, c_int,
                                   c_int64, c_int, c_int, c_float, c_float, c_void_p]),
    "rvc_conv1d_wino_pack_weight": (c_int, [c_void_p, c_int, c_int, c_int, c_void_p, c_void_p]),
    "rvc_conv1d_wino_forward": (c_int, [c_void_p, c_void_p, c_void_p, c_void_p, c_void_p, c_void_p, c_int, c_int, c_int,
                                        c_int64, c_int, c_int, c_float, c_float, c_void_p]),
    "rvc_conv1d_winobf_weight_bytes": (c_int, [c_int, c_int, c_int, POINTER(c_size_t)]),
    "rvc_conv1d_winobf_pack_weight": (c_int, [c_void_p, c_int, c_int, c_int, c_void_p, c_void_p]),
    "rvc_conv1d_winobf_forward": (c_int, [c_void_p, c_void_p, c_void_p, c_void_p, c_void_p, c_void_p, c_int, c_int, c_int,
                                          c_int64, c_int, c_int, c_float, c_float, c_void_p]),
    "rvc_resblock_bf16x3_weight_bytes": (c_int, [c_int, c_int, POINTER(c_size_t)]),
    "rvc_resblock_bf16x3_pack_weight": (c_int, [c_void_p, c_void_p, c_int, c_int, c_void_p, c_void_p]),
    "rvc_resblock_bf16x3_forward": (c_int, [c_void_p, c_void_p, c_void_p, c_void_p, c_void_p, c_void_p, c_int, c_int, c_int64, c_int,
                                            c_int, c_float, c_float, c_void_p]),
    "rvc_resblock_bf16w_weight_bytes": (c_int, [c_int, c_int, POINTER(c_size_t)]),
    "rvc_resblock_bf16w_pack_weight": (c_int, [c_void_p, c_void_p, c_int, c_int, c_void_p, c_void_p]),
    "rvc_resblock_bf16w_forward": (c_int, [c_void_p, c_void_p, c_void_p, c_void_p, c_void_p, c_void_p, c_int, c_int, c_int64, c_int,
                                           c_int, c_float, c_float, c_void_p]),
    "rvc_resblock_bf16x3_set_enabled": (c_int, [c_int]),
    "rvc_upsample_bf16x3_weight_bytes": (c_int, [c_int, c_int, c_int, c_int, c_int, c_int, POINTER(c_size_t)]),
    "rvc_upsample_bf16x3_pack_weight": (c_int, [c_void_p, c_void_p, c_void_p, c_int, c_int, c_int, c_int, c_int, c_int, c_void_p, c_void_p]),
    "rvc_upsample_bf16x3_forward": (c_int, [c_void_p, c_void_p, c_int64, c_void_p, c_void_p, c_void_p, c_int, c_int, c_int, c_int64, c_int, c_int,
                                            c_int, c_int, c_int, c_int, c_float, c_void_p]),
    "rvc_conv1d_f16x2_weight_bytes": (c_int, [c_int, c_int, POINTER(c_size_t)]),
    "rvc_conv1d_f16x2_pack_weight": (c_int, [c_void_p, c_int, c_int, c_void_p, c_void_p]),
    "rvc_conv1d_f16x2_forward": (c_int, [c_void_p, c_void_p, c_void_p, c_void_p, c_void_p, c_void_p, c_int, c_int, c_int64, c_int,
                                         c_int, c_float, c_float, c_void_p]),
    "rvc_decoder_set_arithmetic": (c_int, [c_void_p, c_int]),
    "rvc_conv1d_bf16w_weight_bytes": (c_int, [c_int, c_int, POINTER(c_size_t)]),
    "rvc_conv1d_bf16w_pack_weight": (c_int, [c_void_p, c_int, c_int, c_void_p, c_void_p]),
    "rvc_conv1d_bf16w_forward": (c_int, [c_void_p, c_void_p, c_void_p, c_void_p, c_void_p, c_void_p, c_int, c_int, c_int64, c_int,
                                         c_int, c_float, c_float, c_void_p]),
    "rvc_gemm_bf16x3_weight_bytes": (c_int, [c_int, c_int, POINTER(c_size_t)]),
    "rvc_gemm_bf16x3_pack_weight": (c_int, [c_void_p, c_int, c_int, c_int, c_void_p, c_void_p]),
    "rvc_linear_bf16x3": (c_int, [c_void_p, c_void_p, c_void_p, c_void_p, c_void_p, c_int64, c_int, c_int, c_int, c_void_p]),
    "rvc_conv1d_bf16x3": (c_int, [c_void_p, c_void_p, c_void_p, c_void_p, c_int, c_int, c_int, c_int64, c_int, c_int, c_int, c_int,
                                  c_void_p]),
    "rvc_split_rows_bf16x3": (c_int, [c_void_p, c_void_p, c_int64, c_int64, c_int, c_void_p]),
    "rvc_linear_bf16x3_presplit": (c_int, [c_void_p, c_void_p, c_void_p, c_void_p, c_void_p, c_int64, c_int64, c_int, c_int, c_int, c_int,
                                           c_void_p]),
    "rvc_bias_residual_layernorm_bf16x3": (c_int, [c_void_p, c_int, c_void_p, c_void_p, c_void_p, c_void_p, c_float, c_void_p, c_void_p,
                                                   c_int64, c_int64, c_int, c_void_p]),
    "rvc_conv2d_packed_floats": (c_int, [c_int, c_int, c_int, c_int, POINTER(c_size_t)]),
    "rvc_conv2d_pack_weight": (c_int, [c_void_p, c_int, c_int, c_int, c_int, c_void_p, c_void_p]),
    "rvc_conv2d_workspace_bytes": (c_int, [c_int, c_int, c_int, c_int, c_int, c_int, c_int, POINTER(c_size_t)]),
    "rvc_conv2d_bf16x3_supported": (c_int, [c_int, c_int, c_int, c_int]),
    "rvc_conv2d_bf16x3_weight_bytes": (c_int, [c_int, c_int, c_int, c_int, POINTER(c_size_t)]),
    "rvc_conv2d_bf16x3_pack_weight": (c_int, [c_void_p, c_int, c_int, c_int, c_int, c_void_p, c_void_p]),
    "rvc_conv2d_bf16x3_workspace_bytes": (c_int, [c_int, c_int, c_int, c_int, c_int, POINTER(c_size_t)]),
    "rvc_conv2d_bf16x3_forward": (c_int, [c_void_p, c_void_p, c_void_p, c_void_p, c_void_p, c_int, c_int, c_int, c_int, c_int, c_int,
                                          c_void_p, c_size_t, c_void_p]),
    "rvc_conv2d_forward": (c_int, [c_void_p, c_void_p, c_void_p, c_void_p, c_void_p, c_int, c_int, c_int, c_int, c_int, c_int,
                                   c_int, c_int, c_void_p, c_size_t, c_void_p]),
    "rvc_comm_unique_id": (c_int, [c_void_p]),
    "rvc_comm_create": (c_int, [c_void_p, c_int, c_int, POINTER(c_void_p)]),
    "rvc_comm_destroy": (c_int, [c_void_p]),
    "rvc_comm_info": (c_int, [c_void_p, POINTER(c_int), POINTER(c_int), POINTER(c_int), c_char_p, c_size_t]),
    "rvc_index_broadcast": (c_int, [c_void_p, c_void_p, c_size_t, c_int, c_void_p]),
    "rvc_checksum64": (c_int, [c_void_p, c_size_t, c_void_p, c_void_p]),
    "rvc_glu_dwconv_silu_f32": (c_int, [c_void_p, c_void_p, c_void_p, c_void_p, c_int64, c_int, c_int, c_void_p]),
    "rvc_layernorm_rows_f32": (c_int, [c_void_p, c_void_p, c_void_p, c_float, c_void_p, c_int64, c_int, c_void_p]),
    "rvc_groupnorm_workspace_bytes": (c_int, [c_int, c_int64, c_int, POINTER(c_size_t)]),
    "rvc_groupnorm_lrelu_f32": (c_int, [c_void_p, c_void_p, c_void_p, c_int, c_float, c_float, c_void_p, c_int, c_int64, c_void_p,
                                        c_size_t, c_void_p]),
    "rvc_fcpe_decode_f32": (c_int, [c_void_p, c_void_p, c_int, c_int, c_float, c_float, c_void_p, c_void_p, c_int64, c_void_p]),
    "rvc_kmeans_workspace_bytes": (c_int, [c_int64, c_int64, c_int, POINTER(c_size_t)]),
    "rvc_kmeans_assign": (c_int, [c_void_p, c_int64, c_int, c_void_p, c_int64, c_void_p, c_void_p, c_void_p, c_size_t, c_void_p]),
    "rvc_kmeans_update": (c_int, [c_void_p, c_int64, c_int, c_void_p, c_void_p, c_int64, c_void_p, c_void_p, c_void_p, c_size_t,
                                  c_void_p]),
    "rvc_lfilter_order5_warmup": (c_int, [c_void_p, POINTER(c_int64)]),
    "rvc_lfilter_order5_f64": (c_int, [c_void_p, c_int64, c_void_p, c_void_p, c_void_p]),
    "rvc_frame_rms_frames": (c_int, [c_int64, c_int64, c_int64, POINTER(c_int64), POINTER(c_size_t)]),
    "rvc_frame_rms_f64": (c_int, [c_void_p, c_int64, c_int64, c_int64, c_void_p, c_int64, c_void_p, c_size_t, c_void_p]),
    "rvc_slice_export_f32": (c_int, [c_void_p, c_int64, c_void_p, c_void_p, c_void_p, c_void_p, c_int64, c_int, c_int, c_void_p,
                                     c_int64, c_void_p, c_int64, c_void_p, c_int64, c_void_p]),
    "rvc_spectral_gate_params": (c_int, [c_int, POINTER(c_int), POINTER(c_int), POINTER(ctypes.c_double), c_void_p, c_void_p]),
    "rvc_spectral_gate_workspace_bytes": (c_int, [c_int64, c_int, c_int64, c_int64, POINTER(c_size_t)]),
    "rvc_spectral_gate_f32": (c_int, [c_void_p, c_int64, c_int, c_float, c_int64, c_int64, c_void_p, c_void_p, c_size_t, c_void_p]),
    "rvc_formant_shift_workspace_bytes": (c_int, [c_int64, c_int, POINTER(c_size_t)]),
    "rvc_formant_shift_f32": (c_int, [c_void_p, c_int64, c_int, ctypes.c_double, ctypes.c_double, c_int, c_void_p, c_void_p, c_size_t,
                                      c_void_p]),
    "rvc_mrstft_sums_workspace_bytes": (c_int, [c_int64, POINTER(c_int), POINTER(c_int), POINTER(c_int), c_int, POINTER(c_size_t)]),
    "rvc_mrstft_sums_f32": (c_int, [c_void_p, c_void_p, c_int64, POINTER(c_int), POINTER(c_int), POINTER(c_int), c_int, ctypes.c_double,
                                    c_void_p, c_void_p, c_size_t, c_void_p]),
    "rvc_si_sdr_sums_workspace_bytes": (c_int, [c_int64, POINTER(c_size_t)]),
    "rvc_si_sdr_sums_f32": (c_int, [c_void_p, c_void_p, c_int64, c_void_p, c_void_p, c_size_t, c_void_p]),
    "rvc_mean_abs_diff_workspace_bytes": (c_int, [c_int64, c_int64, POINTER(c_size_t)]),
    "rvc_mean_abs_diff_f32": (c_int, [c_void_p, c_int64, c_void_p, c_int64, c_int64, c_int64, c_void_p, c_void_p, c_size_t, c_void_p]),
    "rvc_sola_workspace_bytes": (c_int, [c_int64, c_int64, POINTER(c_size_t)]),
    "rvc_sola_f32": (c_int, [c_void_p, c_int64, c_void_p, c_void_p, c_int64, c_int64, c_int64, c_void_p, c_void_p, c_void_p, c_size_t,
                             c_void_p]),
    "rvc_stream_window_f32": (c_int, [c_void_p, c_int64, c_void_p, c_int64, c_void_p, c_void_p]),
    "rvc_fx_pointwise_f32": (c_int, [c_void_p, c_int64, c_int, c_double, c_double, c_double, c_double, c_void_p, c_void_p]),
    "rvc_fx_delay_f32": (c_int, [c_void_p, c_int64, c_int, c_double, c_double, c_double, c_void_p, c_void_p]),
    "rvc_fx_chorus_workspace_bytes": (c_int, [c_int64, c_double, POINTER(c_size_t)]),
    "rvc_fx_chorus_f32": (c_int, [c_void_p, c_int64, c_int, c_double, c_double, c_double, c_double, c_double, c_void_p, c_void_p, c_size_t,
                                  c_void_p]),
    "rvc_fx_reverb_params": (c_int, [c_int, POINTER(c_int), POINTER(c_int)]),
    "rvc_fx_reverb_workspace_bytes": (c_int, [c_int64, POINTER(c_size_t)]),
    "rvc_fx_reverb_f32": (c_int, [c_void_p, c_int64, c_int, c_double, c_double, c_double, c_double, c_double, c_double, c_void_p, c_void_p,
                                  c_size_t, c_void_p]),
    "rvc_fx_ballistics": (c_int, [c_int, c_double, c_double, POINTER(c_double), POINTER(c_double)]),
    "rvc_fx_compressor_workspace_bytes": (c_int, [c_int64, c_int64, c_int, POINTER(c_size_t)]),
    "rvc_fx_compressor_f32": (c_int, [c_void_p, c_int64, c_int, c_double, c_double, c_double, c_double, c_int64, c_void_p, c_void_p, c_size_t,
                                      c_void_p]),
    "rvc_fx_limiter_f32": (c_int, [c_void_p, c_int64, c_int, c_double, c_double, c_int64, c_void_p, c_void_p, c_size_t, c_void_p]),
    "rvc_spectral_features_workspace_bytes": (c_int, [c_int64, POINTER(c_size_t)]),
    "rvc_spectral_features_f32": (c_int, [c_void_p, c_int64, c_int, c_double, c_void_p, c_void_p, c_void_p, c_void_p, c_void_p, c_void_p,
                                          c_size_t, c_void_p]),
}

for _name, (_res, _args) in SYMBOLS.items():
    _fn = getattr(_lib, _name)
    _fn.restype = _res
    _fn.argtypes = _args

ABI_VERSION = 4
if _lib.rvc_abi_version() != ABI_VERSION:
    raise ImportError(f"librvc_amd.so ABI {_lib.rvc_abi_version()} != {ABI_VERSION}: rebuild it")


def _check(rc: int, what: str):
    if rc != 0:
        raise NativeError(f"{what}: {_lib.rvc_last_error().decode(errors='replace')}")


def _stream() -> int:
    return torch.cuda.current_stream().cuda_stream


def _call(name: str, device: torch.device, *args, stream: bool = True) -> None:
    if device.index != torch.cuda.current_device():
        if device.type != "cuda" or device.index is None:
            raise NativeError(f"{name}: every tensor must live in HBM, got one on {device}")
        with torch.cuda.device(device):
            return _call(name, device, *args, stream=stream)
    if stream:
        args += (torch.cuda.current_stream(device.index).cuda_stream,)
    _check(getattr(_lib, name)(*args), name)


def _device(*tensors) -> torch.device:
    device = None
    for t in tensors:
        if t is None:
            continue
        if device is None:
            device = t.device
        elif t.device != device:
            raise NativeError(f"the tensors of one call must share a device, got {device} and {t.device}")
    return device


def _cuda_device(device=None) -> torch.device:
    device = torch.device("cuda" if device is None else device)
    if device.type != "cuda":
        raise NativeError(f"a HIP device is needed, got {device} (no CPU fallback)")
    return device if device.index is not None else torch.device("cuda", torch.cuda.current_device())


def _ptr(t):
    return t.data_ptr() if t is not None else None


def _host(w: torch.Tensor) -> torch.Tensor:
    return w.detach().float().cpu().contiguous()


def _dev_f32(t: torch.Tensor, name: str) -> torch.Tensor:
    if not t.is_cuda:
        raise NativeError(f"{name} must live in HBM (got a {t.device} tensor); the HIP path has no CPU fallback")
    if t.dtype != torch.float32:
        raise NativeError(f"{name} must be float32, got {t.dtype}")
    return t.contiguous()


class _Workspace:

    def __init__(self):
        self._buf = {}
        self._lock = threading.Lock()
# ... 525 lines not shown
    return out


def bigru_redone(batch: int = 1, device=None) -> int:
    device = _cuda_device(device)
    ws = _workspace("bigru", device, "rvc_bigru_workspace_bytes", batch)
    n = c_int()
    _call("rvc_bigru_status", device, ws.data_ptr(), batch, ctypes.byref(n))
    return n.value


def bigru_set_spin_limit(polls: int) -> None:
    _check(_lib.rvc_bigru_set_spin_limit(int(polls)), "rvc_bigru_set_spin_limit")


def _is_f32_hbm(t: torch.Tensor) -> bool:
    return t.is_cuda and t.dtype == torch.float32 and t.is_contiguous()


def attention_qkv(qkv: torch.Tensor, n_heads: int, scale: float, emb_rel_k: torch.Tensor = None,
                  emb_rel_v: torch.Tensor = None) -> torch.Tensor:
    if not (_is_f32_hbm(qkv) and qkv.dim() == 3):
        raise NativeError("attention_qkv wants a contiguous float32 HBM tensor [B, T, 3 * n_heads * d]")
    b, t, c = qkv.shape
    hd = c // (3 * n_heads)
    rel = (emb_rel_k, emb_rel_v) if emb_rel_k is not None else (None, None)
    if rel[0] is not None and not all(e is not None and _is_f32_hbm(e) and tuple(e.shape) == (21, hd) for e in rel):
        raise NativeError(f"attention_qkv wants emb_rel_k and emb_rel_v as contiguous float32 HBM tensors [21, {hd}]")
    dev = _device(qkv, *rel)
    out = torch.empty(b, t, n_heads * hd, dtype=torch.float32, device=dev)
    ws = _workspace("attention", dev, "rvc_attention_workspace_bytes", b, t, n_heads, hd)
    _call("rvc_attention_qkv_f32", dev, qkv.data_ptr(), _ptr(rel[0]), _ptr(rel[1]), out.data_ptr(), b, t, n_heads, hd, float(scale),
          ws.data_ptr(), ws.numel())
    return out


def bias_relu_add_(x: torch.Tensor, bias: torch.Tensor = None, res: torch.Tensor = None, relu: bool = True) -> torch.Tensor:
    if not (_is_f32_hbm(x) and x.dim() >= 3):
        raise NativeError("bias_relu_add_ wants a contiguous float32 HBM tensor [B, C, ...]")
    b, c = x.shape[0], x.shape[1]
    inner = x.numel() // (b * c)
    if res is not None and not (_is_f32_hbm(res) and res.shape == x.shape):
        raise NativeError("bias_relu_add_ wants res as a contiguous float32 HBM tensor of x's shape")
    _call("rvc_bias_relu_add_f32", _device(x, bias, res), x.data_ptr(), _ptr(bias), _ptr(res), x.data_ptr(), b, c, inner, int(relu))
    return x


def rownorm_gelu_(x: torch.Tensor, gamma: torch.Tensor = None, beta: torch.Tensor = None, eps: float = 1e-5) -> torch.Tensor:
    if not (_is_f32_hbm(x) and x.dim() == 3):
        raise NativeError("rownorm_gelu_ wants a contiguous float32 HBM tensor [B, C, L]")
    b, c, length = x.shape
    _call("rvc_rownorm_gelu_f32", _device(x, gamma, beta), x.data_ptr(), _ptr(gamma), _ptr(beta), x.data_ptr(), b, c, length, float(eps))
    return x


def gate_tanh_sigmoid(x: torch.Tensor) -> torch.Tensor:
    if not (_is_f32_hbm(x) and x.dim() == 3 and x.shape[1] % 2 == 0):
        raise NativeError("gate_tanh_sigmoid wants a contiguous float32 HBM tensor [B, 2H, T]")
    b, c2, t = x.shape
    out = torch.empty(b, c2 // 2, t, dtype=torch.float32, device=x.device)
    _call("rvc_gate_tanh_sigmoid_f32", x.device, x.data_ptr(), out.data_ptr(), b, c2 // 2, t)
    return out


def set_concurrency_hint(utterances_in_flight: int) -> None:
    _check(_lib.rvc_set_concurrency_hint(int(utterances_in_flight)), "rvc_set_concurrency_hint")


COMM_ID_BYTES = 128


def comm_unique_id() -> bytes:
    buf = ctypes.create_string_buffer(COMM_ID_BYTES)
    _check(_lib.rvc_comm_unique_id(buf), "rvc_comm_unique_id")
    return buf.raw


class Comm:

    def __init__(self, unique_id: bytes, n_ranks: int, rank: int):
        if len(unique_id) != COMM_ID_BYTES:
            raise NativeError(f"Comm wants the {COMM_ID_BYTES}-byte id of comm_unique_id, got {len(unique_id)} bytes")
        self._h = c_void_p()
        _check(_lib.rvc_comm_create(ctypes.create_string_buffer(unique_id, COMM_ID_BYTES), int(n_ranks), int(rank),
                                    ctypes.byref(self._h)), "rvc_comm_create")

    def info(self) -> dict:
        n, r, v = c_int(), c_int(), c_int()
        path = ctypes.create_string_buffer(512)
        _check(_lib.rvc_comm_info(self._h, ctypes.byref(n), ctypes.byref(r), ctypes.byref(v), path, 512), "rvc_comm_info")
        return {"n_ranks": n.value, "rank": r.value, "rccl_version": v.value, "library": path.value.decode()}

    def broadcast_(self, t: torch.Tensor, root: int = 0) -> torch.Tensor:
        if not t.is_cuda or not t.is_contiguous():
            raise NativeError("Comm.broadcast_ wants a contiguous HBM tensor")
        _call("rvc_index_broadcast", t.device, self._h, t.data_ptr(), t.numel() * t.element_size(), int(root))
        return t

    def destroy(self):
        h, self._h = self._h, None
        if h:
            _check(_lib.rvc_comm_destroy(h), "rvc_comm_destroy")

    def __del__(self):
        if getattr(self, "_h", None) and _lib is not None:
            _lib.rvc_comm_destroy(self._h)
            self._h = None


def checksum64(t: torch.Tensor) -> torch.Tensor:
    if not t.is_cuda or not t.is_contiguous():
        raise NativeError("checksum64 wants a contiguous HBM tensor")
    out = torch.empty(2, dtype=torch.int64, device=t.device)
    _call("rvc_checksum64", t.device, t.data_ptr(), t.numel() * t.element_size(), out.data_ptr())
    return out


def conv1d_pack_weight(w: torch.Tensor, device) -> torch.Tensor:
    w = _host(w)
    packed = torch.empty(w.numel(), dtype=torch.float32, device=device)
    _call("rvc_conv1d_pack_weight", packed.device, w.data_ptr(), w.shape[0], w.shape[1], w.shape[2], packed.data_ptr())
    return packed


def conv1d_wino_pack_weight(w: torch.Tensor, device) -> torch.Tensor:
    w = _host(w)
    c_out, c_in, k = w.shape
    u = torch.empty(3 * ((k + 2) // 3) * c_in * c_out, dtype=torch.float32, device=device)
    _call("rvc_conv1d_wino_pack_weight", u.device, w.data_ptr(), c_out, c_in, k, u.data_ptr())
    return u


def conv1d_winobf_pack_weight(w: torch.Tensor, device) -> torch.Tensor:
    w = _host(w)
    return _pack_slab("rvc_conv1d_winobf", device, (w,), tuple(w.shape))


def _conv1d_square_pack(stem: str, w: torch.Tensor, device) -> torch.Tensor:
    w = _host(w)
    c, c_in, k = w.shape
    if c != c_in:
        raise NativeError(f"{stem[4:]}: a square conv expected, got {tuple(w.shape)}")
    return _pack_slab(stem, device, (w,), (c, k))


def conv1d_bf16w_pack_weight(w: torch.Tensor, device) -> torch.Tensor:
    return _conv1d_square_pack("rvc_conv1d_bf16w", w, device)


def conv1d_f16x2_pack_weight(w: torch.Tensor, device) -> torch.Tensor:
    return _conv1d_square_pack("rvc_conv1d_f16x2", w, device)


def _conv1d(name: str, x, w_packed, bias, c_out, k, dilation, slope_in, res, acc, out_scale, out):
    x = _dev_f32(x, "x")
    b, c_in, length = x.shape
    square = c_out is None
    y = out if out is not None else torch.empty((b, c_in if square else c_out, length), dtype=torch.float32, device=x.device)
    if square and y.data_ptr() == x.data_ptr():
        raise NativeError(f"{name[4:-8]}: x and y must not alias")
    _call(name, _device(x, w_packed, bias, res, acc, y), x.data_ptr(), w_packed.data_ptr(), _ptr(bias), _ptr(res), _ptr(acc), y.data_ptr(),
          b, *((c_in,) if square else (c_in, c_out)), length, k, dilation, float(slope_in), float(out_scale))
    return y


def conv1d_forward(x, w_packed, bias, c_out, k, dilation=1, slope_in=1.0, res=None, acc=None, out_scale=1.0):
    return _conv1d("rvc_conv1d_forward", x, w_packed, bias, c_out, k, dilation, slope_in, res, acc, out_scale, None)


def conv1d_forward_into(x, w_packed, bias, c_out, k, dilation=1, slope_in=1.0, res=None, acc=None, out_scale=1.0, out=None):
    return _conv1d("rvc_conv1d_forward", x, w_packed, bias, c_out, k, dilation, slope_in, res, acc, out_scale, out)


def conv1d_wino_forward(x, u_packed, bias, c_out, k, dilation=1, slope_in=1.0, res=None, acc=None, out_scale=1.0, out=None):
    return _conv1d("rvc_conv1d_wino_forward", x, u_packed, bias, c_out, k, dilation, slope_in, res, acc, out_scale, out)


def conv1d_winobf_forward(x, u_packed, bias, c_out, k, dilation=1, slope_in=1.0, res=None, acc=None, out_scale=1.0, out=None):
    return _conv1d("rvc_conv1d_winobf_forward", x, u_packed, bias, c_out, k, dilation, slope_in, res, acc, out_scale, out)


def conv1d_bf16w_forward(x, u_packed, bias, k, dilation=1, slope_in=1.0, res=None, acc=None, out_scale=1.0, out=None):
    return _conv1d("rvc_conv1d_bf16w_forward", x, u_packed, bias, None, k, dilation, slope_in, res, acc, out_scale, out)


def conv1d_f16x2_forward(x, u_packed, bias, k, dilation=1, slope_in=1.0, res=None, acc=None, out_scale=1.0, out=None):
    return _conv1d("rvc_conv1d_f16x2_forward", x, u_packed, bias, None, k, dilation, slope_in, res, acc, out_scale, out)


def resblock_bf16x3_pack_weight(w1: torch.Tensor, w2: torch.Tensor, device, bf16_taps: bool = False) -> torch.Tensor:
    w1, w2 = _host(w1), _host(w2)
    c, c_in, k = w1.shape
    if c != c_in or w2.shape != w1.shape:
        raise NativeError(f"resblock pair: square convs of one shape expected, got {tuple(w1.shape)} and {tuple(w2.shape)}")
    return _pack_slab("rvc_resblock_bf16w" if bf16_taps else "rvc_resblock_bf16x3", device, (w1, w2), (c, k))


def resblock_bf16x3_forward(x, u_packed, b1, b2, k, dilation=1, slope=0.1, acc=None, out_scale=1.0, out=None, bf16_taps: bool = False):
    x = _dev_f32(x, "x")
    b, c, length = x.shape
    y = out if out is not None else torch.empty_like(x)
    if y.data_ptr() == x.data_ptr():
        raise NativeError("resblock pair: x and y must not alias")
    _call("rvc_resblock_bf16w_forward" if bf16_taps else "rvc_resblock_bf16x3_forward", _device(x, u_packed, b1, b2, acc, y),
          x.data_ptr(), u_packed.data_ptr(), _ptr(b1), _ptr(b2), _ptr(acc), y.data_ptr(), b, c, length, k, dilation, float(slope),
          float(out_scale))
    return y


def upsample_bf16x3_pack_weight(up_w: torch.Tensor, noise_w, bias, rate: int, nc_stride: int, device):
    up_w = _host(up_w)
    c_in, c_out, ksize = up_w.shape
    nw = _host(noise_w).reshape(c_out, -1).contiguous() if noise_w is not None else None
    nc_k = nw.shape[1] if nw is not None else 0
    b = _host(bias) if bias is not None else None
    u = _pack_slab("rvc_upsample_bf16x3", device, (up_w, nw, b), (c_in, c_out, rate, ksize, nc_k, nc_stride))
    return u, (nw.to(device) if nw is not None else None), (b.to(device) if b is not None else None)


def upsample_bf16x3_forward(x, har, packed, c_out, rate, ksize, pad, nc_stride=1, nc_pad=0, slope=0.1):
    u, nw, bias = packed
    x = _dev_f32(x, "x")
    b, c_in, length = x.shape
    l_out = (length - 1) * rate - 2 * pad + ksize
    y = torch.empty((b, c_out, l_out), dtype=torch.float32, device=x.device)
    if har is not None:
        har = _dev_f32(har, "har")
    _call("rvc_upsample_bf16x3_forward", _device(x, har, u, bias), x.data_ptr(), _ptr(har), har.shape[-1] if har is not None else 0,
          u.data_ptr(), _ptr(bias), y.data_ptr(), b, c_in, c_out, length, rate, ksize, pad, nw.shape[1] if nw is not None else 0,
          nc_stride, nc_pad, float(slope))
    return y


def resblock_bf16x3_set_enabled(enabled: bool) -> None:
    _check(_lib.rvc_resblock_bf16x3_set_enabled(1 if enabled else 0), "rvc_resblock_bf16x3_set_enabled")


def gemm_bf16x3_pack_weight(w: torch.Tensor, device) -> torch.Tensor:
    w = _host(w)
    taps = w.shape[2] if w.dim() == 3 else 1
    m, k_total = w.shape[0], w.shape[1] * taps
    return _pack_slab("rvc_gemm_bf16x3", device, (w,), (m, k_total), (m, k_total, taps))


def linear_bf16x3(x: torch.Tensor, a_packed: torch.Tensor, bias, out_features: int, act: str = "none", res=None) -> torch.Tensor:
    x = _dev_f32(x, "x")
    in_features = x.shape[-1]
    n_rows = x.numel() // in_features
    y = torch.empty(x.shape[:-1] + (out_features,), dtype=torch.float32, device=x.device)
    if res is not None:
        res = _dev_f32(res, "res")
        if res.shape != y.shape:
            raise NativeError(f"linear_bf16x3: res {tuple(res.shape)} must have the result's shape {tuple(y.shape)}")
    _call("rvc_linear_bf16x3", _device(x, a_packed, bias, res), x.data_ptr(), a_packed.data_ptr(), _ptr(bias), _ptr(res), y.data_ptr(),
          n_rows, in_features, out_features, {"none": 0, "gelu": 1}[act])
    return y


def glu_dwconv_silu(x: torch.Tensor, w: torch.Tensor, bias: torch.Tensor) -> torch.Tensor:
    x, w, bias = _dev_f32(x, "x"), _dev_f32(w, "w"), _dev_f32(bias, "bias")
    n_rows, c = x.shape[0], x.shape[1] // 2
    y = torch.empty((n_rows, c), dtype=torch.float32, device=x.device)
    _call("rvc_glu_dwconv_silu_f32", _device(x, w, bias), x.data_ptr(), w.data_ptr(), bias.data_ptr(), y.data_ptr(), n_rows, c, w.shape[1])
    return y


def layernorm_rows(x: torch.Tensor, gamma: torch.Tensor, beta: torch.Tensor, eps: float = 1e-5) -> torch.Tensor:
    x, gamma, beta = _dev_f32(x, "x"), _dev_f32(gamma, "gamma"), _dev_f32(beta, "beta")
    f = x.shape[-1]
    y = torch.empty_like(x)
    _call("rvc_layernorm_rows_f32", _device(x, gamma, beta), x.data_ptr(), gamma.data_ptr(), beta.data_ptr(), float(eps), y.data_ptr(),
          x.numel() // f, f)
    return y


def groupnorm_lrelu(x: torch.Tensor, gamma: torch.Tensor, beta: torch.Tensor, groups: int, eps: float = 1e-5,
                    slope: float = 0.01) -> torch.Tensor:
    x = _dev_f32(x, "x")
    c, length = x.shape
    ws = _workspace("groupnorm", x.device, "rvc_groupnorm_workspace_bytes", c, length, groups)
    y = torch.empty_like(x)
    gamma, beta = _dev_f32(gamma, "gamma"), _dev_f32(beta, "beta")
    _call("rvc_groupnorm_lrelu_f32", _device(x, gamma, beta), x.data_ptr(), gamma.data_ptr(), beta.data_ptr(), groups, float(eps),
          float(slope), y.data_ptr(), c, length, ws.data_ptr(), ws.numel())
    return y


def fcpe_decode(logits: torch.Tensor, cent_table: torch.Tensor, out_dims: int, threshold: float, f0_min: float,
                want_latent: bool = False):
    logits, cent_table = _dev_f32(logits, "logits"), _dev_f32(cent_table, "cent_table")
    n_rows, ld = logits.shape
    if cent_table.numel() != out_dims:
        raise NativeError(f"cent_table has {cent_table.numel()} entries, out_dims is {out_dims}")
    dev = _device(logits, cent_table)
    f0 = torch.empty(n_rows, dtype=torch.float32, device=dev)
    latent = torch.empty((n_rows, out_dims), dtype=torch.float32, device=dev) if want_latent else None
    _call("rvc_fcpe_decode_f32", dev, logits.data_ptr(), cent_table.data_ptr(), out_dims, ld, float(threshold), float(f0_min),
          f0.data_ptr(), _ptr(latent), n_rows)
    return f0, latent


def rows_padded(n_rows: int, tile: int = 128) -> int:
    return -(-n_rows // tile) * tile


def planes_empty(n_rows: int, features: int, device) -> torch.Tensor:
    return torch.empty((3, rows_padded(n_rows), features), dtype=torch.bfloat16, device=device)


def split_rows_bf16x3(x: torch.Tensor, out: torch.Tensor | None = None) -> torch.Tensor:
    x = _dev_f32(x, "x")
    n_rows, k = x.shape
    xs = out if out is not None else planes_empty(n_rows, k, x.device)
    _call("rvc_split_rows_bf16x3", _device(x, xs), x.data_ptr(), xs.data_ptr(), n_rows, xs.shape[1], k)
    return xs


def linear_bf16x3_presplit(xs: torch.Tensor, a_packed: torch.Tensor, bias, n_rows: int, out_features: int, mode: str = "f32",
                           k_parts: int = 1, out: torch.Tensor | None = None) -> torch.Tensor:
    _, n_pad, in_features = xs.shape
    m = {"f32": 0, "gelu_planes": 1, "parts": 2, "gelu_f32": 3}[mode]
    if m in (0, 3):
        y = out if out is not None else torch.empty((n_rows, out_features), dtype=torch.float32, device=xs.device)
    elif m == 1:
        y = out if out is not None else torch.empty((3, n_pad, out_features), dtype=torch.bfloat16, device=xs.device)
    else:
        y = out if out is not None else torch.empty((k_parts, n_rows, out_features), dtype=torch.float32, device=xs.device)
    _call("rvc_linear_bf16x3_presplit", _device(xs, a_packed, bias, y), xs.data_ptr(), a_packed.data_ptr(), _ptr(bias),
          y.data_ptr() if m != 1 else None, y.data_ptr() if m == 1 else None, n_rows, n_pad, in_features, out_features, m, k_parts)
    return y


def posconv_bf16x3_pack_weight(w: torch.Tensor, groups: int, device) -> torch.Tensor:
    w = _host(w)
    return _pack_slab("rvc_posconv_bf16x3", device, (w,), (w.shape[0], groups, w.shape[2]))

# ... 215 lines not shown
```

include/rvc_amd.h:

```cpp
#ifndef RVC_AMD_H
#define RVC_AMD_H

#include <stddef.h>
#include <stdint.h>

#ifdef __cplusplus
extern "C" {
#endif

#define RVC_AMD_ABI_VERSION 4


int rvc_abi_version(void);
const char *rvc_last_error(void);


int rvc_knn_index_aux_bytes(int64_t n_rows, int dim, size_t *bytes);
int rvc_knn_index_build(const float *index_dev, int64_t n_rows, int dim, void *aux_dev, size_t aux_bytes, void *stream);

int rvc_knn_workspace_bytes(int64_t n_rows, int64_t n_queries, int dim, int k, size_t *bytes);

int rvc_knn_search(const float *index_dev, const void *aux_dev, int64_t n_rows, int dim,
                   const float *queries_dev, int64_t n_queries, int k,
                   float *out_d2_dev, int64_t *out_ids_dev,
// ... 14 lines not shown
                     int64_t n_frames_padded, void *workspace_dev, size_t workspace_bytes, void *stream);

typedef struct rvc_mel rvc_mel;
int rvc_mel_create(int n_fft, int hop, int win_length, int pad, float mag_eps, float log_floor, const float *mel_host, int n_mels,
                   rvc_mel **out);
int rvc_mel_destroy(rvc_mel *h);
int rvc_mel_frames(const rvc_mel *h, int64_t n_samples, int64_t *n_frames);
int rvc_mel_workspace_bytes(const rvc_mel *h, int batch, int64_t n_samples, size_t *bytes);
int rvc_mel_forward(const rvc_mel *h, const float *audio_dev, int batch, int64_t n_samples, float *mel_dev, float *spec_dev,
                    void *workspace_dev, size_t workspace_bytes, void *stream);

int rvc_resample_poly_f64(const double *x_dev, int64_t n_in, int up, int down, const double *h_dev, int64_t n_taps,
                          double *y_dev, int64_t n_out, void *stream);

int rvc_filtfilt_workspace_bytes(int64_t n, size_t *bytes);
int rvc_filtfilt_order5(const double *x_dev, int64_t n, const double *coef_host, double *y_dev,
                        void *workspace_dev, size_t workspace_bytes, void *stream);

int rvc_bigru_workspace_bytes(int batch, size_t *bytes);
int rvc_bigru_status(const void *workspace_dev, int batch, int *n_redone_host, void *stream);
int rvc_bigru_set_spin_limit(unsigned polls);
int rvc_bigru_forward(const float *gi_dev, const float *whhT_dev, const float *bhh_dev, float *out_dev,
                      int batch, int64_t n_steps, int hidden, void *workspace_dev, size_t workspace_bytes, void *stream);

int rvc_attention_workspace_bytes(int batch, int64_t n_frames, int n_heads, int head_dim, size_t *bytes);
int rvc_attention_qkv_f32(const float *qkv_dev, const float *emb_rel_k_dev, const float *emb_rel_v_dev, float *out_dev,
                          int batch, int64_t n_frames, int n_heads, int head_dim, float scale, void *workspace_dev,
                          size_t workspace_bytes, void *stream);

int rvc_bias_relu_add_f32(const float *x_dev, const float *bias_dev, const float *res_dev, float *out_dev, int batch,
                          int channels, int64_t inner, int relu, void *stream);

int rvc_rownorm_gelu_f32(const float *x_dev, const float *gamma_dev, const float *beta_dev, float *out_dev, int batch, int channels,
                         int64_t length, float eps, void *stream);

int rvc_gate_tanh_sigmoid_f32(const float *x_dev, float *out_dev, int batch, int hidden, int64_t length, void *stream);

int rvc_set_concurrency_hint(int utterances_in_flight);

typedef struct rvc_decoder rvc_decoder;

enum { RVC_DEC_NSF = 0, RVC_DEC_MRF = 1, RVC_DEC_REFINE = 2 };

typedef struct rvc_decoder_config {
    int kind;
    int sample_rate;
    int in_channels;
    int upsample_initial_channel;
    int gin_channels;
    int n_ups;
    int upsample_rates[8];
    int upsample_kernel_sizes[8];
    int n_res_kernels;
    int res_kernel_sizes[4];
    int res_dilations[4];
    int n_res_dilations;
    int weight_storage;
} rvc_decoder_config;

int rvc_decoder_create(const rvc_decoder_config *cfg, rvc_decoder **out);
int rvc_decoder_set_tensor(rvc_decoder *dec, const char *name, const float *data_host,
                           const int64_t *shape, int ndim);
int rvc_decoder_finalize(rvc_decoder *dec);
int rvc_decoder_destroy(rvc_decoder *dec);

int rvc_decoder_upp(const rvc_decoder *dec);
int rvc_decoder_workspace_bytes(const rvc_decoder *dec, int batch, int64_t n_frames, size_t *bytes);

typedef struct rvc_decoder_noise {
    const float *src_rand_dev;
    const float *src_randn_dev;
    const float *adain_randn_dev;
} rvc_decoder_noise;

int rvc_decoder_forward(rvc_decoder *dec, const float *z_dev, const float *f0_dev, const float *g_dev,
                        const rvc_decoder_noise *noise, int batch, int64_t n_frames, float *out_dev,
                        void *workspace_dev, size_t workspace_bytes, void *stream);

int rvc_decoder_window_margin(const rvc_decoder_config *cfg, int *frames);
int rvc_decoder_forward_window(rvc_decoder *dec, const float *z_dev, const float *f0_dev, const float *g_dev,
                               const rvc_decoder_noise *noise, int batch, int64_t n_frames, int64_t keep_lo, int64_t keep_hi,
                               float *out_dev, void *workspace_dev, size_t workspace_bytes, void *stream);

int rvc_decoder_set_concurrency_hint(rvc_decoder *dec, int utterances_in_flight);

int rvc_decoder_set_branch_parallel(rvc_decoder *dec, int side_streams);

int rvc_decoder_set_arithmetic(rvc_decoder *dec, int mode);

int rvc_decoder_set_tap(rvc_decoder *dec, int stage, float *tap_dev);

int rvc_conv1d_pack_weight(const float *w_host, int c_out, int c_in, int k, float *w_packed_dev, void *stream);
int rvc_conv1d_forward(const float *x_dev, const float *w_packed_dev, const float *bias_dev,
                       const float *res_dev, const float *acc_dev, float *y_dev,
                       int batch, int c_in, int c_out, int64_t length, int k, int dilation,
                       float slope_in, float out_scale, void *stream);

typedef struct rvc_comm rvc_comm;
#define RVC_COMM_ID_BYTES 128
int rvc_comm_unique_id(unsigned char *id_host );
int rvc_comm_create(const unsigned char *id_host, int n_ranks, int rank, rvc_comm **out);
int rvc_comm_destroy(rvc_comm *comm);
int rvc_comm_info(const rvc_comm *comm, int *n_ranks, int *rank, int *rccl_version, char *library_path,
                  size_t library_path_bytes);
int rvc_index_broadcast(rvc_comm *comm, void *buf_dev, size_t bytes, int root, void *stream);
int rvc_checksum64(const void *buf_dev, size_t bytes, uint64_t *out2_dev, void *stream);

int rvc_conv2d_packed_floats(int c_out, int c_in, int kh, int kw, size_t *out);
int rvc_conv2d_pack_weight(const float *w_host, int c_out, int c_in, int kh, int kw, float *w_dev, void *stream);
int rvc_conv2d_workspace_bytes(int batch, int c_in, int c_out, int height, int width, int kh, int kw, size_t *out);
int rvc_conv2d_forward(const float *x_dev, const float *w_packed_dev, const float *bias_dev, const float *res_dev,
                       float *y_dev, int batch, int c_in, int c_out, int height, int width, int kh, int kw, int relu,
                       void *workspace_dev, size_t workspace_bytes, void *stream);

int rvc_conv2d_bf16x3_supported(int c_in, int c_out, int height, int width);
int rvc_conv2d_bf16x3_weight_bytes(int c_out, int c_in, int kh, int kw, size_t *bytes);
int rvc_conv2d_bf16x3_pack_weight(const float *w_host, int c_out, int c_in, int kh, int kw, void *u_dev, void *stream);
int rvc_conv2d_bf16x3_workspace_bytes(int batch, int c_in, int c_out, int height, int width, size_t *out);
int rvc_conv2d_bf16x3_forward(const float *x_dev, const void *u_dev, const float *bias_dev, const float *res_dev, float *y_dev,
                              int batch, int c_in, int c_out, int height, int width, int relu, void *workspace_dev,
                              size_t workspace_bytes, void *stream);

int rvc_conv1d_wino_pack_weight(const float *w_host, int c_out, int c_in, int k, float *u_dev, void *stream);
int rvc_conv1d_wino_forward(const float *x_dev, const float *u_dev, const float *bias_dev, const float *res_dev,
                            const float *acc_dev, float *y_dev, int batch, int c_in, int c_out, int64_t length, int k,
                            int dilation, float slope_in, float out_scale, void *stream);

int rvc_conv1d_winobf_weight_bytes(int c_out, int c_in, int k, size_t *bytes);
int rvc_conv1d_winobf_pack_weight(const float *w_host, int c_out, int c_in, int k, void *u_dev, void *stream);
int rvc_conv1d_winobf_forward(const float *x_dev, const void *u_dev, const float *bias_dev, const float *res_dev,
                              const float *acc_dev, float *y_dev, int batch, int c_in, int c_out, int64_t length, int k,
                              int dilation, float slope_in, float out_scale, void *stream);

int rvc_resblock_bf16x3_weight_bytes(int c, int k, size_t *bytes);
int rvc_resblock_bf16x3_pack_weight(const float *w1_host, const float *w2_host, int c, int k, void *u_dev, void *stream);
int rvc_resblock_bf16x3_forward(const float *x_dev, const void *u_dev, const float *b1_dev, const float *b2_dev,
                                const float *acc_dev, float *y_dev, int batch, int c, int64_t length, int k, int dilation,
                                float slope, float out_scale, void *stream);
int rvc_resblock_bf16w_weight_bytes(int c, int k, size_t *bytes);
int rvc_resblock_bf16w_pack_weight(const float *w1_host, const float *w2_host, int c, int k, void *u_dev, void *stream);
int rvc_resblock_bf16w_forward(const float *x_dev, const void *u_dev, const float *b1_dev, const float *b2_dev,
                               const float *acc_dev, float *y_dev, int batch, int c, int64_t length, int k, int dilation,
                               float slope, float out_scale, void *stream);
int rvc_conv1d_bf16w_weight_bytes(int c, int k, size_t *bytes);
int rvc_conv1d_bf16w_pack_weight(const float *w_host, int c, int k, void *u_dev, void *stream);
int rvc_conv1d_bf16w_forward(const float *x_dev, const void *u_dev, const float *bias_dev, const float *res_dev,
                             const float *acc_dev, float *y_dev, int batch, int c, int64_t length, int k, int dilation,
                             float slope_in, float out_scale, void *stream);
int rvc_conv1d_f16x2_weight_bytes(int c, int k, size_t *bytes);
int rvc_conv1d_f16x2_pack_weight(const float *w_host, int c, int k, void *u_dev, void *stream);
int rvc_conv1d_f16x2_forward(const float *x_dev, const void *u_dev, const float *bias_dev, const float *res_dev,
                             const float *acc_dev, float *y_dev, int batch, int c, int64_t length, int k, int dilation,
                             float slope_in, float out_scale, void *stream);
int rvc_upsample_bf16x3_weight_bytes(int c_in, int c_out, int rate, int ksize, int nc_k, int nc_stride, size_t *bytes);
int rvc_upsample_bf16x3_pack_weight(const float *up_w_host, const float *noise_w_host, const float *bias_host, int c_in, int c_out,
                                    int rate, int ksize, int nc_k, int nc_stride, void *u_dev, void *stream);
int rvc_upsample_bf16x3_forward(const float *x_dev, const float *har_dev, int64_t har_len, const void *u_dev, const float *bias_dev,
                                float *y_dev, int batch, int c_in, int c_out, int64_t length_in, int rate, int ksize, int pad,
                                int nc_k, int nc_stride, int nc_pad, float slope_in, void *stream);
int rvc_resblock_bf16x3_set_enabled(int enabled);

int rvc_gemm_bf16x3_weight_bytes(int m, int k_total, size_t *bytes);
int rvc_gemm_bf16x3_pack_weight(const float *w_host, int m, int k_total, int conv_taps, void *a_dev, void *stream);
int rvc_linear_bf16x3(const float *x_dev, const void *a_dev, const float *bias_dev, const float *res_dev, float *y_dev,
                      int64_t n_rows, int in_features, int out_features, int act, void *stream);
int rvc_conv1d_bf16x3(const float *x_dev, const void *a_dev, const float *bias_dev, float *y_dev, int batch, int c_in,
                      int c_out, int64_t l_in, int k, int stride, int padding, int act, void *stream);

int rvc_split_rows_bf16x3(const float *x_dev, void *xs_dev, int64_t n_rows, int64_t n_rows_padded, int k, void *stream);
int rvc_linear_bf16x3_presplit(const void *xs_dev, const void *a_dev, const float *bias_dev, float *y_dev, void *ys_dev,
                               int64_t n_rows, int64_t n_rows_padded, int in_features, int out_features, int mode, int k_parts,
                               void *stream);
int rvc_bias_residual_layernorm_bf16x3(const float *parts_dev, int n_parts, const float *bias_dev, const float *res_dev,
                                       const float *gamma_dev, const float *beta_dev, float eps, float *y_dev, void *ys_dev,
                                       int64_t n_rows, int64_t n_rows_padded, int features, void *stream);

int rvc_hubert_conv0_workspace_bytes(int channels, size_t *bytes);
int rvc_hubert_conv0_frames_bf16x3(const float *wav_dev, int64_t n_samples, const float *w_dev, int channels, int taps, int stride,
                                   const float *gamma_dev, const float *beta_dev, float eps, void *workspace_dev,
                                   size_t workspace_bytes, void *ys_dev, int64_t n_frames_padded, void *stream);
int rvc_conv1d_frames_bf16x3(const void *xs_dev, int64_t n_frames_in, int64_t n_frames_in_padded, int channels, int taps, int stride,
                             const void *a_dev, const float *bias_dev, float *y_dev, void *ys_dev, int64_t n_frames_out_padded,
                             int out_channels, int mode, void *stream);

int rvc_posconv_bf16x3_weight_bytes(int d, int groups, int taps, size_t *bytes);
int rvc_posconv_bf16x3_pack_weight(const float *w_host, int d, int groups, int taps, void *a_dev, void *stream);
int rvc_posconv_gelu_bf16x3(const float *x_dev, const void *a_dev, const float *bias_dev, float *y_dev, int64_t n_frames, int d,
                            int groups, int taps, int padding, void *stream);

int rvc_glu_dwconv_silu_f32(const float *x_dev, const float *w_dev, const float *bias_dev, float *y_dev, int64_t n_rows, int C, int K,
                            void *stream);
int rvc_layernorm_rows_f32(const float *x_dev, const float *gamma_dev, const float *beta_dev, float eps, float *y_dev, int64_t n_rows,
                           int F, void *stream);
int rvc_groupnorm_workspace_bytes(int C, int64_t L, int groups, size_t *bytes);
int rvc_groupnorm_lrelu_f32(const float *x_dev, const float *gamma_dev, const float *beta_dev, int groups, float eps, float slope,
                            float *y_dev, int C, int64_t L, void *workspace_dev, size_t workspace_bytes, void *stream);
int rvc_fcpe_decode_f32(const float *logits_dev, const float *cent_table_dev, int out_dims, int ld, float threshold, float f0_min,
                        float *f0_dev, float *latent_dev, int64_t n_rows, void *stream);

int rvc_kmeans_workspace_bytes(int64_t n_rows, int64_t n_centroids, int dim, size_t *bytes);
int rvc_kmeans_assign(const float *x_dev, int64_t n_rows, int dim, const float *centroids_dev, int64_t n_centroids,
                      int32_t *out_ids_dev, float *out_d2_dev, void *workspace_dev, size_t workspace_bytes, void *stream);
int rvc_kmeans_update(const float *x_dev, int64_t n_rows, int dim, const int32_t *order_dev, const int64_t *offsets_dev,
                      int64_t n_centroids, const float *old_centroids_dev, float *out_centroids_dev, void *workspace_dev,
                      size_t workspace_bytes, void *stream);

int rvc_lfilter_order5_warmup(const double *coef_host, int64_t *warm);
int rvc_lfilter_order5_f64(const double *x_dev, int64_t n, const double *coef_host, double *y_dev, void *stream);
int rvc_frame_rms_frames(int64_t n, int64_t frame_length, int64_t hop, int64_t *n_frames, size_t *workspace_bytes);
int rvc_frame_rms_f64(const double *x_dev, int64_t n, int64_t frame_length, int64_t hop, double *out_dev, int64_t n_frames,
                      void *workspace_dev, size_t workspace_bytes, void *stream);
int rvc_slice_export_f32(const double *x_dev, int64_t n, const int64_t *bounds_host, const int64_t *seg_dev,
                         const int64_t *off_full_dev, const int64_t *off_lo_dev, int64_t n_seg, int up, int down,
                         const double *h_dev, int64_t n_taps, float *full_dev, int64_t n_full, float *lo_dev, int64_t n_lo,
                         void *stream);

int rvc_spectral_gate_params(int sr, int *nf, int *nt, double *b, double *freq_taps, double *time_taps);
int rvc_spectral_gate_workspace_bytes(int64_t n, int sr, int64_t chunk_size, int64_t padding, size_t *bytes);
int rvc_spectral_gate_f32(const float *y_dev, int64_t n, int sr, float prop_decrease, int64_t chunk_size, int64_t padding,
                          float *out_dev, void *workspace_dev, size_t workspace_bytes, void *hip_stream);

int rvc_formant_shift_workspace_bytes(int64_t n, int group_frames, size_t *bytes);
int rvc_formant_shift_f32(const float *x_dev, int64_t n, int sr, double quefrency_s, double distortion, int group_frames,
                          float *out_dev, void *workspace_dev, size_t workspace_bytes, void *hip_stream);

int rvc_mrstft_sums_workspace_bytes(int64_t n, const int *n_fft, const int *hop, const int *win, int n_res, size_t *bytes);
int rvc_mrstft_sums_f32(const float *x_dev, const float *y_dev, int64_t n, const int *n_fft, const int *hop, const int *win, int n_res,
                        double eps, double *out_dev, void *workspace_dev, size_t workspace_bytes, void *hip_stream);
int rvc_si_sdr_sums_workspace_bytes(int64_t n, size_t *bytes);
int rvc_si_sdr_sums_f32(const float *preds_dev, const float *target_dev, int64_t n, double *out_dev, void *workspace_dev,
                        size_t workspace_bytes, void *hip_stream);
int rvc_mean_abs_diff_workspace_bytes(int64_t rows, int64_t min_t, size_t *bytes);
int rvc_mean_abs_diff_f32(const float *a_dev, int64_t a_stride, const float *b_dev, int64_t b_stride, int64_t rows, int64_t min_t,
                          double *out_dev, void *workspace_dev, size_t workspace_bytes, void *hip_stream);

int rvc_sola_workspace_bytes(int64_t xfade, int64_t search, size_t *bytes);
int rvc_sola_f32(const float *infer_dev, int64_t n_infer, float *buf_dev, const float *fade_in_dev, int64_t xfade, int64_t search,
                 int64_t block, float *out_dev, int *offset_dev, void *workspace_dev, size_t workspace_bytes, void *hip_stream);
int rvc_stream_window_f32(float *hist_dev, int64_t n_hist, const float *block_dev, int64_t n_block, float *window_dev,
                          void *hip_stream);

int rvc_fx_pointwise_f32(const float *x_dev, int64_t n, int stages, double gain_db, double drive_db, double bit_depth,
                         double clip_threshold_db, float *out_dev, void *hip_stream);
int rvc_fx_delay_f32(const float *x_dev, int64_t n, int sr, double delay_seconds, double feedback, double mix, float *out_dev,
                     void *hip_stream);
int rvc_fx_chorus_workspace_bytes(int64_t n, double feedback, size_t *bytes);
int rvc_fx_chorus_f32(const float *x_dev, int64_t n, int sr, double rate_hz, double depth, double centre_delay_ms, double feedback,
                      double mix, float *out_dev, void *workspace_dev, size_t workspace_bytes, void *hip_stream);
int rvc_fx_reverb_params(int sr, int *comb_len, int *allpass_len);
int rvc_fx_reverb_workspace_bytes(int64_t n, size_t *bytes);
int rvc_fx_reverb_f32(const float *x_dev, int64_t n, int sr, double room_size, double damping, double wet_level, double dry_level,
                      double width, double freeze_mode, float *out_dev, void *workspace_dev, size_t workspace_bytes, void *hip_stream);
int rvc_fx_ballistics(int sr, double attack_ms, double release_ms, double *c_attack, double *c_release);
int rvc_fx_compressor_workspace_bytes(int64_t n, int64_t chunk, int limiter, size_t *bytes);
int rvc_fx_compressor_f32(const float *x_dev, int64_t n, int sr, double threshold_db, double ratio, double attack_ms,
                          double release_ms, int64_t chunk, float *out_dev, void *workspace_dev, size_t workspace_bytes,
                          void *hip_stream);
int rvc_fx_limiter_f32(const float *x_dev, int64_t n, int sr, double threshold_db, double release_ms, int64_t chunk, float *out_dev,
                       void *workspace_dev, size_t workspace_bytes, void *hip_stream);

int rvc_spectral_features_workspace_bytes(int64_t n, size_t *bytes);
int rvc_spectral_features_f32(const float *x_dev, int64_t n, int sr, double roll_percent, float *mag_dev, float *db_dev,
                              double *cent_dev, double *bw_dev, double *rolloff_dev, void *workspace_dev, size_t workspace_bytes,
                              void *hip_stream);

#ifdef __cplusplus
}
#endif
#endif
```

Before: 62.00 million.

## Add bf16x3 direct conv path for 256-channel k3 vocoder ResBlock convs

Adds a third fragment format to the direct square-conv kernel that packs each weight as three bf16 planes and issues six split products per tap, keeping fp32-accurate results. In the default fp32 arithmetic mode, 256-channel kernel-3 ResBlock convs now route to this kernel ahead of the Winograd bf16 path. Bias is folded in by the stager waves. It uses more weight memory and more MFMA work per output than Winograd in exchange for skipping the transform overhead, and it adds a launch counter and ABI entry points.

After: 59.07 million. -4.7%, worse.

```diff
diff --git a/codename-rvc-fork-3_amd/csrc/conv.h b/codename-rvc-fork-3_amd/csrc/conv.h
--- a/codename-rvc-fork-3_amd/csrc/conv.h
+++ b/codename-rvc-fork-3_amd/csrc/conv.h
@@ -30,6 +30,7 @@
     const uint32_t *w_wino16 = nullptr;
     const void *w_f16x2 = nullptr;
     const void *w_direct1 = nullptr;
+    const void *w_direct3 = nullptr;
     const void *w_winobf = nullptr;
     const float *w_wino = nullptr;
     int debug = 0;
@@ -60,8 +61,10 @@
 enum Cb1Format {
     CB1_BF16W = 0,
     CB1_F16X2 = 1,
+    CB1_BF16X3 = 2,
 };
 bool convbf1_supported(int c, int k, int dil);
+bool convbf1_supported(Cb1Format fmt, int c, int k, int dil);
 bool convbf1_preferred(Cb1Format fmt, int c, int k);
 bool convbf1_fits(int c, int64_t L);
 size_t convbf1_weight_bytes(Cb1Format fmt, int c, int k);
diff --git a/codename-rvc-fork-3_amd/csrc/conv.hip b/codename-rvc-fork-3_amd/csrc/conv.hip
--- a/codename-rvc-fork-3_amd/csrc/conv.hip
+++ b/codename-rvc-fork-3_amd/csrc/conv.hip
@@ -407,6 +407,10 @@
         convbf1_fits(p_in.c1, p_in.l_in))
         return launch_convbf1(p_in.w_f16x2 ? CB1_F16X2 : CB1_BF16W, p_in.x1, p_in.w_f16x2 ? p_in.w_f16x2 : p_in.w_direct1, p_in.bias, p_in.res, p_in.accin,
                               p_in.y, p_in.batch, p_in.c1, p_in.l_out, p_in.kw, p_in.dil, p_in.slope1, p_in.out_scale, stream);
+    if (p_in.w_direct3 && plain && p_in.c1 == p_in.m_total && p_in.x1 != p_in.y && convbf1_supported(CB1_BF16X3, p_in.c1, p_in.kw, p_in.dil) &&
+        convbf1_fits(p_in.c1, p_in.l_in))
+        return launch_convbf1(CB1_BF16X3, p_in.x1, p_in.w_direct3, p_in.bias, p_in.res, p_in.accin, p_in.y, p_in.batch, p_in.c1, p_in.l_out, p_in.kw,
+                              p_in.dil, p_in.slope1, p_in.out_scale, stream);
     if (p_in.w_winobf && plain && wino_enabled() && winobf_enabled() && winobf_supported(p_in.c1, p_in.m_total, p_in.kw, p_in.dil) &&
         winobf_fits(p_in.c1, p_in.m_total, p_in.l_in))
         return launch_winobf_conv(p_in.x1, p_in.w_winobf, p_in.bias, p_in.res, p_in.accin, p_in.y, p_in.batch, p_in.c1, p_in.m_total, p_in.l_out,
diff --git a/codename-rvc-fork-3_amd/csrc/convbf1.hip b/codename-rvc-fork-3_amd/csrc/convbf1.hip
--- a/codename-rvc-fork-3_amd/csrc/convbf1.hip
+++ b/codename-rvc-fork-3_amd/csrc/convbf1.hip
@@ -1,6 +1,7 @@
 #include <stdlib.h>
 
 #include <algorithm>
+#include <atomic>
 #include <mutex>
 #include <type_traits>
 #include <vector>
@@ -21,6 +22,9 @@
     static constexpr int PLANES = 3;
     static constexpr int TAPF = 1;
     static constexpr int NACC = 1;
+    static constexpr int NTERMS = 3;
+    static constexpr int RING256 = 8;
+    static constexpr bool STAGER_BIAS = false;
     static constexpr int OUT_OPS = 24, VM_MAX = 56;
     static constexpr int tap_plane(int) { return 0; }
     static constexpr int win_plane(int i) { return 2 - i; }
@@ -33,10 +37,29 @@
     static constexpr int PLANES = 2;
     static constexpr int TAPF = 2;
     static constexpr int NACC = 2;
+    static constexpr int NTERMS = 3;
+    static constexpr int RING256 = 4;
+    static constexpr bool STAGER_BIAS = true;
     static constexpr int OUT_OPS = 28, VM_MAX = 60;
     static constexpr int tap_plane(int i) { return i == 2; }
     static constexpr int win_plane(int i) { return i == 0; }
     static constexpr int acc_of(int i) { return i != 1; }
+};
+
+struct Cb1Bf16x3 {
+    static constexpr const char *NAME = "convbf3";
+    using frag = bf16x8;
+    static constexpr bool PAIRS = false;
+    static constexpr int PLANES = 3;
+    static constexpr int TAPF = 3;
+    static constexpr int NACC = 1;
+    static constexpr int NTERMS = 6;
+    static constexpr int RING256 = 3;
+    static constexpr bool STAGER_BIAS = true;
+    static constexpr int OUT_OPS = 28, VM_MAX = 60;
+    static constexpr int tap_plane(int i) { return i < 3 ? i : i == 4; }
+    static constexpr int win_plane(int i) { return i < 3 ? 2 - i : i == 3; }
+    static constexpr int acc_of(int) { return 0; }
 };
 
 struct Cb1Params {
@@ -69,7 +92,7 @@
     static constexpr int LDS_BYTES = 2 * X_BYTES + IO_BYTES;
     static constexpr int ROWBLOCKS = C / 32;
     static constexpr int CONV_BYTES = NGT * ROWBLOCKS * F::TAPF * 1024;
-    static constexpr int PA = F::TAPF == 1 ? 8 : 8 / RBW;
+    static constexpr int PA = RBW == 1 ? 8 : F::RING256;
     static_assert(C == 128 || C == 256, "square layers of 128 or 256 channels");
     static_assert((CB1_CK / 8) * RC32 % 4 == 0, "the items must divide over the four stager waves");
     static_assert(4 * NIT + F::OUT_OPS <= F::VM_MAX, "memory operations in flight per stager wave");
@@ -187,7 +210,7 @@
                     const unsigned o = o0 + (unsigned)((hf * HP + k) * 4 * RPW) * L4;
                     rv[k] = f32x4{0.f, 0.f, 0.f, 0.f};
                     av[k] = f32x4{0.f, 0.f, 0.f, 0.f};
-                    if constexpr (F::PAIRS)
+                    if constexpr (F::STAGER_BIAS)
                         bv[k] = __builtin_bit_cast(float, __builtin_amdgcn_raw_buffer_load_b32(brs, (int)(has_bias ? (unsigned)((((hf * HP + k) * 4 + sw) * RPW + rsub) * 4) : BUF_OOB), 0, 0));
                     if (has_res) rv[k] = load4(rrs, o);
                     if (has_acc) av[k] = load4(ars, o);
@@ -201,7 +224,7 @@
                     const float r4[4] = {rv[k].x, rv[k].y, rv[k].z, rv[k].w}, a4[4] = {av[k].x, av[k].y, av[k].z, av[k].w};
 #pragma unroll
                     for (int e = 0; e < 4; ++e) {
-                        if constexpr (F::PAIRS) re[e] = add_np(re[e], bv[k]);
+                        if constexpr (F::STAGER_BIAS) re[e] = add_np(re[e], bv[k]);
                         if (has_res) re[e] = add_np(re[e], r4[e]);
                         if (has_acc) re[e] = add_np(re[e], a4[e]);
                         re[e] = mul_np(re[e], out_scale);
@@ -234,7 +257,7 @@
     }
 
     float bias[RBW][16];
-    if constexpr (!F::PAIRS) {
+    if constexpr (!F::STAGER_BIAS) {
 #pragma unroll
         for (int rb = 0; rb < RBW; ++rb)
 #pragma unroll
@@ -265,7 +288,7 @@
     for (int g = 0; g < PA - 1; ++g) load_a(g, g);
     const int x_lane = l31 * ROWB + half * 16;
     float *const io_mine = io_lds + (32 * RBW * wave + 4 * half) * N1 + l31;
-    constexpr int NM = 6 * RBW;
+    constexpr int NM = 2 * F::NTERMS * RBW;
 
     static_assert((2 * NGC) % PA == 0 && NCH % 2 == 0, "two chunks of groups must be whole turns of the tap ring");
     int q = 0;
@@ -291,7 +314,7 @@
                 for (int gc = 0; gc < NGC; ++gc) {
                     const int gl = c2 * NGC + gc;
 #pragma unroll
-                    for (int i = 0; i < 3; ++i)
+                    for (int i = 0; i < F::NTERMS; ++i)
 #pragma unroll
                         for (int cb = 0; cb < 2; ++cb)
 #pragma unroll
@@ -322,6 +345,8 @@
                 for (int r = 0; r < 16; ++r)
                     if constexpr (F::PAIRS)
                         io_mine[(32 * rb + (r & 3) + 8 * (r >> 2)) * N1 + cb * 32] = __builtin_fmaf(acc[rb][cb][1][r], F16X2_LO_UNSCALE, acc[rb][cb][0][r]);
+                    else if constexpr (F::STAGER_BIAS)
+                        io_mine[(32 * rb + (r & 3) + 8 * (r >> 2)) * N1 + cb * 32] = acc[rb][cb][0][r];
                     else
                         io_mine[(32 * rb + (r & 3) + 8 * (r >> 2)) * N1 + cb * 32] = acc[rb][cb][0][r] + bias[rb][r];
     }
@@ -329,9 +354,18 @@
 }
 
 
+static std::atomic<uint64_t> cb3_launches{0};
+
 bool convbf1_supported(int c, int k, int dil) { return (c == 128 || c == 256) && (k == 3 || k == 7 || k == 11) && dil >= 1 && dil <= 5; }
-
+bool convbf1_supported(Cb1Format fmt, int c, int k, int dil) {
+    return fmt == CB1_BF16X3 ? c == 256 && k == 3 && dil >= 1 && dil <= 5 : convbf1_supported(c, k, dil);
+}
+static const char *cb1_name(Cb1Format fmt) { return fmt == CB1_F16X2 ? Cb1F16Pairs::NAME : fmt == CB1_BF16X3 ? Cb1Bf16x3::NAME : Cb1Bf16Taps::NAME; }
+static int cb1_planes(Cb1Format fmt) { return fmt == CB1_F16X2 ? Cb1F16Pairs::TAPF : fmt == CB1_BF16X3 ? Cb1Bf16x3::TAPF : Cb1Bf16Taps::TAPF; }
+
+constexpr bool CB3_SELECTED = true;
 bool convbf1_preferred(Cb1Format fmt, int c, int k) {
+    if (fmt == CB1_BF16X3) return CB3_SELECTED && convbf1_supported(fmt, c, k, 1);
     if (fmt == CB1_F16X2) {
 #ifdef RVC_ABLATE
         static const int on = knob("RVC_CH2", 1);
@@ -350,10 +384,10 @@
 
 bool convbf1_fits(int c, int64_t L) { return fits_2gib((int64_t)c * L, 4); }
 
-size_t convbf1_weight_bytes(Cb1Format fmt, int c, int k) { return (size_t)(c / 16) * k * (c / 32) * 1024 * (fmt == CB1_F16X2 ? 2 : 1); }
+size_t convbf1_weight_bytes(Cb1Format fmt, int c, int k) { return (size_t)(c / 16) * k * (c / 32) * 1024 * cb1_planes(fmt); }
 
 int convbf1_pack_host(Cb1Format fmt, const float *w, int c, int k, std::vector<uint16_t> *out) {
-    const int NCH = c / CB1_CK, KS = CB1_CK / 16, RB = c / 32, planes = fmt == CB1_F16X2 ? 2 : 1;
+    const int NCH = c / CB1_CK, KS = CB1_CK / 16, RB = c / 32, planes = cb1_planes(fmt);
     if (fmt == CB1_F16X2)
         for (size_t i = 0, n = (size_t)c * c * k; i < n; ++i)
             if (!(w[i] >= -F16_MAX && w[i] <= F16_MAX)) return 1;
@@ -368,7 +402,11 @@
                             const size_t group = ((size_t)ch * k + tap) * KS + ks, at = (group * RB + rb) * planes * 512 + lane * 8 + e;
                             const float v = w[((size_t)co * c + ci) * k + tap];
                             if (fmt == CB1_F16X2) f16x2_split_host(v, &(*out)[at], &(*out)[at + 512]);
-                            else (*out)[at] = bf16_rne(v);
+                            else if (fmt == CB1_BF16X3) {
+                                uint16_t h[3];
+                                bf16_split_host(v, 3, h);
+                                for (int s = 0; s < 3; ++s) (*out)[at + s * 512] = h[s];
+                            } else (*out)[at] = bf16_rne(v);
                         }
     return 0;
 }
@@ -396,8 +434,8 @@
 
 int launch_convbf1(Cb1Format fmt, const float *x, const void *u, const float *bias, const float *res, const float *accin, float *y, int batch,
                    int c, int64_t L, int k, int dil, float slope, float out_scale, hipStream_t stream) {
-    const char *const name = fmt == CB1_F16X2 ? Cb1F16Pairs::NAME : Cb1Bf16Taps::NAME;
-    if (!convbf1_supported(c, k, dil)) return fail("%s: unsupported shape (%d channels, %d taps, dilation %d)", name, c, k, dil);
+    const char *const name = cb1_name(fmt);
+    if (!convbf1_supported(fmt, c, k, dil)) return fail("%s: unsupported shape (%d channels, %d taps, dilation %d)", name, c, k, dil);
     if (x == y) return fail("%s: in-place operation is not supported", name);
     if (!(slope >= 0.f && slope <= 1.f)) return fail("%s: leaky slope %g outside [0, 1]", name, (double)slope);
     if (!convbf1_fits(c, L)) return fail("%s: a %d x %lld slab exceeds the 2 GiB buffer addressing", name, c, (long long)L);
@@ -405,6 +443,10 @@
     if ((int64_t)ceil_div(L, CB1_N1) * batch >= ((int64_t)1 << 28)) return fail("%s: too many tiles", name);
     Cb1Params p;
     p.x = x; p.u = u; p.bias = bias; p.res = res; p.accin = accin; p.y = y; p.L = L; p.dil = dil; p.slope = slope; p.out_scale = out_scale;
+    if (fmt == CB1_BF16X3) {
+        cb3_launches.fetch_add(1, std::memory_order_relaxed);
+        return cb1_launch<3, 256, Cb1Bf16x3>(p, batch, stream);
+    }
     return fmt == CB1_F16X2 ? cb1_dispatch<Cb1F16Pairs>(p, batch, c, k, stream) : cb1_dispatch<Cb1Bf16Taps>(p, batch, c, k, stream);
 }
 
@@ -415,6 +457,7 @@
 
 static int cb1_abi_weight_bytes(Cb1Format fmt, const char *fn, int c, int k, size_t *bytes) {
     if (!bytes) return fail("%s: null pointer", fn);
+    if (fmt == CB1_BF16X3 && !convbf1_supported(fmt, c, k, 1)) return fail("%s: c must be 256 and k 3", fn);
     if (!convbf1_supported(c, k, 1)) return fail("%s: c must be 128 or 256, k 3, 7 or 11", fn);
     *bytes = convbf1_weight_bytes(fmt, c, k);
     return 0;
@@ -462,3 +505,31 @@
     return cb1_abi_forward(CB1_F16X2, "rvc_conv1d_f16x2_forward", x_dev, u_dev, bias_dev, res_dev, acc_dev, y_dev, batch, c, length, k,
                            dilation, slope_in, out_scale, stream);
 }
+
+extern "C" int rvc_conv1d_bf16x3d_weight_bytes(int c, int k, size_t *bytes) {
+    return cb1_abi_weight_bytes(CB1_BF16X3, "rvc_conv1d_bf16x3d_weight_bytes", c, k, bytes);
+}
+extern "C" int rvc_conv1d_bf16x3d_pack_weight(const float *w_host, int c, int k, void *u_dev, void *stream) {
+    return cb1_abi_pack_weight(CB1_BF16X3, "rvc_conv1d_bf16x3d_pack_weight", "rvc_conv1d_bf16x3d_pack_weight", w_host, c, k, u_dev, stream);
+}
+extern "C" int rvc_conv1d_bf16x3d_forward(const float *x_dev, const void *u_dev, const float *bias_dev, const float *res_dev,
+                                          const float *acc_dev, float *y_dev, int batch, int c, int64_t length, int k, int dilation,
+                                          float slope_in, float out_scale, void *stream) {
+    return cb1_abi_forward(CB1_BF16X3, "rvc_conv1d_bf16x3d_forward", x_dev, u_dev, bias_dev, res_dev, acc_dev, y_dev, batch, c, length, k,
+                           dilation, slope_in, out_scale, stream);
+}
+extern "C" int rvc_conv1d_bf16x3d_pack_weight_host(const float *w_host, int c, int k, void *u_host) {
+    const char *const fn = "rvc_conv1d_bf16x3d_pack_weight_host";
+    if (!w_host || !u_host) return fail("%s: null pointer", fn);
+    size_t bytes = 0;
+    if (cb1_abi_weight_bytes(CB1_BF16X3, fn, c, k, &bytes)) return 1;
+    std::vector<uint16_t> u;
+    convbf1_pack_host(CB1_BF16X3, w_host, c, k, &u);
+    memcpy(u_host, u.data(), bytes);
+    return 0;
+}
+extern "C" int rvc_conv1d_bf16x3d_launches(uint64_t *count) {
+    if (!count) return fail("rvc_conv1d_bf16x3d_launches: null pointer");
+    *count = cb3_launches.load(std::memory_order_relaxed);
+    return 0;
+}
diff --git a/codename-rvc-fork-3_amd/csrc/decoder.h b/codename-rvc-fork-3_amd/csrc/decoder.h
--- a/codename-rvc-fork-3_amd/csrc/decoder.h
+++ b/codename-rvc-fork-3_amd/csrc/decoder.h
@@ -39,6 +39,7 @@
     DevBuf16 wx;
     DevBuf16 wd;
     DevBuf16 wh;
+    DevBuf16 wt;
     int c_in = 0, c_out = 0, k = 0;
 };
 
diff --git a/codename-rvc-fork-3_amd/csrc/decoder.hip b/codename-rvc-fork-3_amd/csrc/decoder.hip
--- a/codename-rvc-fork-3_amd/csrc/decoder.hip
+++ b/codename-rvc-fork-3_amd/csrc/decoder.hip
@@ -428,6 +428,11 @@
             if (d->arithmetic == 1 && convbf1_supported(c_out, k, 1) && convbf1_preferred(CB1_F16X2, c_out, k)) {
                 std::vector<uint16_t> frags;
                 if (!convbf1_pack_host(CB1_F16X2, w->data.data(), c_out, k, &frags) && out->wh.upload(frags)) return 1;
+            }
+            if (d->arithmetic == 0 && d->cfg.kind != RVC_DEC_REFINE && convbf1_supported(CB1_BF16X3, c_out, k, 1) && convbf1_preferred(CB1_BF16X3, c_out, k)) {
+                std::vector<uint16_t> frags;
+                convbf1_pack_host(CB1_BF16X3, w->data.data(), c_out, k, &frags);
+                if (out->wt.upload(frags)) return 1;
             }
             if (winobf_enabled() && winobf_supported(c_in, c_out, k, 1)) {
                 std::vector<uint16_t> frags;
@@ -950,14 +955,14 @@
                 const int dil = c.res_dilations[j];
                 ConvParams p;
                 p.x1 = xin; p.c1 = s.c_out; p.slope1 = 0.1f; p.x1_bstride = bs; p.l_in = len;
-                p.w = s.c1[m * nd + j].w.p; p.w16 = s.c1[m * nd + j].w16.p; p.bias = s.c1[m * nd + j].b.p; p.w_wino = s.c1[m * nd + j].wu.p; p.w_winobf = s.c1[m * nd + j].wx.p; p.w_direct1 = s.c1[m * nd + j].wd.p; p.w_f16x2 = s.c1[m * nd + j].wh.p;
+                p.w = s.c1[m * nd + j].w.p; p.w16 = s.c1[m * nd + j].w16.p; p.bias = s.c1[m * nd + j].b.p; p.w_wino = s.c1[m * nd + j].wu.p; p.w_winobf = s.c1[m * nd + j].wx.p; p.w_direct1 = s.c1[m * nd + j].wd.p; p.w_f16x2 = s.c1[m * nd + j].wh.p; p.w_direct3 = s.c1[m * nd + j].wt.p;
                 p.w_wino16 = reinterpret_cast<const uint32_t *>(s.c1[m * nd + j].wu16.p);
                 p.y = T1; p.y_bstride = bs; p.m_total = s.c_out; p.c_out = s.c_out; p.n_cols = len; p.l_out = len;
                 p.kw = k; p.dil = dil; p.padl = (k - 1) / 2 * dil; p.batch = batch;
                 if (launch_conv(p, stream)) return 1;
                 ConvParams q;
                 q.x1 = T1; q.c1 = s.c_out; q.slope1 = 0.1f; q.x1_bstride = bs; q.l_in = len;
-                q.w = s.c2[m * nd + j].w.p; q.w16 = s.c2[m * nd + j].w16.p; q.bias = s.c2[m * nd + j].b.p; q.w_wino = s.c2[m * nd + j].wu.p; q.w_winobf = s.c2[m * nd + j].wx.p; q.w_direct1 = s.c2[m * nd + j].wd.p; q.w_f16x2 = s.c2[m * nd + j].wh.p;
+                q.w = s.c2[m * nd + j].w.p; q.w16 = s.c2[m * nd + j].w16.p; q.bias = s.c2[m * nd + j].b.p; q.w_wino = s.c2[m * nd + j].wu.p; q.w_winobf = s.c2[m * nd + j].wx.p; q.w_direct1 = s.c2[m * nd + j].wd.p; q.w_f16x2 = s.c2[m * nd + j].wh.p; q.w_direct3 = s.c2[m * nd + j].wt.p;
                 q.w_wino16 = reinterpret_cast<const uint32_t *>(s.c2[m * nd + j].wu16.p);
                 q.res = xin;
                 q.y_bstride = bs; q.m_total = s.c_out; q.c_out = s.c_out; q.n_cols = len; q.l_out = len;
diff --git a/codename-rvc-fork-3_amd/rvc_amd/_native.py b/codename-rvc-fork-3_amd/rvc_amd/_native.py
--- a/codename-rvc-fork-3_amd/rvc_amd/_native.py
+++ b/codename-rvc-fork-3_amd/rvc_amd/_native.py
@@ -124,6 +124,12 @@
     "rvc_conv1d_f16x2_forward": (c_int, [c_void_p, c_void_p, c_void_p, c_void_p, c_void_p, c_void_p, c_int, c_int, c_int64, c_int,
                                          c_int, c_float, c_float, c_void_p]),
     "rvc_decoder_set_arithmetic": (c_int, [c_void_p, c_int]),
+    "rvc_conv1d_bf16x3d_weight_bytes": (c_int, [c_int, c_int, POINTER(c_size_t)]),
+    "rvc_conv1d_bf16x3d_pack_weight": (c_int, [c_void_p, c_int, c_int, c_void_p, c_void_p]),
+    "rvc_conv1d_bf16x3d_forward": (c_int, [c_void_p, c_void_p, c_void_p, c_void_p, c_void_p, c_void_p, c_int, c_int, c_int64, c_int,
+                                           c_int, c_float, c_float, c_void_p]),
+    "rvc_conv1d_bf16x3d_pack_weight_host": (c_int, [c_void_p, c_int, c_int, c_void_p]),
+    "rvc_conv1d_bf16x3d_launches": (c_int, [POINTER(ctypes.c_uint64)]),
     "rvc_conv1d_bf16w_weight_bytes": (c_int, [c_int, c_int, POINTER(c_size_t)]),
     "rvc_conv1d_bf16w_pack_weight": (c_int, [c_void_p, c_int, c_int, c_void_p, c_void_p]),
     "rvc_conv1d_bf16w_forward": (c_int, [c_void_p, c_void_p, c_void_p, c_void_p, c_void_p, c_void_p, c_int, c_int, c_int64, c_int,
@@ -955,6 +961,16 @@
     return _conv1d_square_pack("rvc_conv1d_f16x2", w, device)
 
 
+def conv1d_bf16x3d_pack_weight(w: torch.Tensor, device) -> torch.Tensor:
+    return _conv1d_square_pack("rvc_conv1d_bf16x3d", w, device)
+
+
+def conv1d_bf16x3d_launches() -> int:
+    n = ctypes.c_uint64()
+    _check(_lib.rvc_conv1d_bf16x3d_launches(ctypes.byref(n)), "rvc_conv1d_bf16x3d_launches")
+    return int(n.value)
+
+
 def _conv1d(name: str, x, w_packed, bias, c_out, k, dilation, slope_in, res, acc, out_scale, out):
     x = _dev_f32(x, "x")
     b, c_in, length = x.shape
@@ -985,6 +1001,10 @@
 
 def conv1d_bf16w_forward(x, u_packed, bias, k, dilation=1, slope_in=1.0, res=None, acc=None, out_scale=1.0, out=None):
     return _conv1d("rvc_conv1d_bf16w_forward", x, u_packed, bias, None, k, dilation, slope_in, res, acc, out_scale, out)
+
+
+def conv1d_bf16x3d_forward(x, u_packed, bias, k, dilation=1, slope_in=1.0, res=None, acc=None, out_scale=1.0, out=None):
+    return _conv1d("rvc_conv1d_bf16x3d_forward", x, u_packed, bias, None, k, dilation, slope_in, res, acc, out_scale, out)
 
 
 def conv1d_f16x2_forward(x, u_packed, bias, k, dilation=1, slope_in=1.0, res=None, acc=None, out_scale=1.0, out=None):
diff --git a/include/rvc_amd.h b/include/rvc_amd.h
--- a/include/rvc_amd.h
+++ b/include/rvc_amd.h
@@ -190,6 +190,13 @@
 int rvc_conv1d_f16x2_forward(const float *x_dev, const void *u_dev, const float *bias_dev, const float *res_dev,
                              const float *acc_dev, float *y_dev, int batch, int c, int64_t length, int k, int dilation,
                              float slope_in, float out_scale, void *stream);
+int rvc_conv1d_bf16x3d_weight_bytes(int c, int k, size_t *bytes);
+int rvc_conv1d_bf16x3d_pack_weight(const float *w_host, int c, int k, void *u_dev, void *hip_stream);
+int rvc_conv1d_bf16x3d_forward(const float *x_dev, const void *u_dev, const float *bias_dev, const float *res_dev,
+                               const float *acc_dev, float *y_dev, int batch, int c, int64_t length, int k, int dilation,
+                               float slope_in, float out_scale, void *hip_stream);
+int rvc_conv1d_bf16x3d_pack_weight_host(const float *w_host, int c, int k, void *u_host);
+int rvc_conv1d_bf16x3d_launches(uint64_t *count);
 int rvc_upsample_bf16x3_weight_bytes(int c_in, int c_out, int rate, int ksize, int nc_k, int nc_stride, size_t *bytes);
 int rvc_upsample_bf16x3_pack_weight(const float *up_w_host, const float *noise_w_host, const float *bias_host, int c_in, int c_out,
                                     int rate, int ksize, int nc_k, int nc_stride, void *u_dev, void *stream);
```
